# the-byte-bender/GraphAudio

Hardware: AMD Instinct MI355X
Metric: rendered frames/sec @48kHz, 1024-voice convolver graph (higher is better)
Workload: dtype f32

## Files before the change

graphaudio_amd/csrc/ga_api.cpp:

```cpp
#include <algorithm>
#include <cstring>

#include <execinfo.h>
#include <signal.h>
#include <unistd.h>

#include "ga_engine.hpp"

using namespace ga;

static void ga_segv_handler(int sig) {
  void* frames[64];
  int n = backtrace(frames, 64);
  const char msg[] = "\n[graphaudio_hip] fatal signal, native backtrace:\n";
  (void)!write(2, msg, sizeof(msg) - 1);
  backtrace_symbols_fd(frames, n, 2);
  signal(sig, SIG_DFL);
  raise(sig);
}
__attribute__((constructor)) static void ga_install_handler() {
  const char* e = getenv("GA_BACKTRACE");
  if (e && e[0] == '1') signal(SIGSEGV, ga_segv_handler);
}

struct ga_context {
  Context c;
  explicit ga_context(int sr) : c(sr) {}
};

namespace {
template <class F>
int guardRO(ga_context* h, F&& f) {
  if (!h) return GA_ERR_INVALID_ARGUMENT;
  try {
    f(h->c);
    return GA_OK;
  } catch (const Err& e) {
    h->c.lastError = e.msg;
    return e.code;
  } catch (const std::bad_alloc&) {
    h->c.lastError = "out of host memory";
    return GA_ERR_OUT_OF_MEMORY;
  } catch (const std::exception& e) {
    h->c.lastError = e.what();
    return GA_ERR_INVALID_OPERATION;
  } catch (...) {
    h->c.lastError = "unknown error";
    return GA_ERR_INVALID_OPERATION;
  }
}
template <class F>
int guard(ga_context* h, F&& f) {
  if (h) h->c.apiEpoch++;
  return guardRO(h, std::forward<F>(f));
}
float clampf(float v, float mn, float mx) {
  if (v < mn) return mn;
  if (v > mx) return mx;
  return v;
}
void addEvent(ParamS& p, const ParamEvent& e) {
  size_t lo = 0, hi = p.events.size();
  while (lo < hi) {
    size_t mid = (lo + hi) >> 1;
    if (e.time < p.events[mid].time) hi = mid; else lo = mid + 1;
  }
  p.events.insert(p.events.begin() + lo, e);
}
}

int64_t Context::chunkLimit(int64_t) {
    int64_t limit = maxChunkBlocks;
    {
      size_t freeB = 0, totalB = 0;
      if (hipMemGetInfo(&freeB, &totalB) == hipSuccess) {
        double perBlock = 0, fixedBytes = 0;
        int convRowsMax = 0;
        for (auto& g : groups) convRowsMax = std::max(convRowsMax, (int)((g->rows.size() + 127) / 128 * 128));
        perBlock += (double)convRowsMax * kBins * 4.0 * 4.0;
        int tailMax = kCoarseMaxP;
        for (auto& np : nodes)
          if (np->type == GA_NODE_CONVOLVER)
            if (const ConvolverS& cv = rec<ConvolverS>(*np); cv.ir && cv.convPath == 4) tailMax = std::max(tailMax, cv.ir->coarseP);
        for (auto& np : nodes) {
          if (np->type != GA_NODE_CONVOLVER) continue;
          const ConvolverS& cv = rec<ConvolverS>(*np);
          if (cv.ir && cv.convPath == 4) {
// ... 12 lines not shown
        budget += (double)(coarseX.bytes + coarseY.bytes + coarseM.bytes);
        int64_t byMem = (int64_t)(std::max(budget - fixedBytes, 0.0) / std::max(perBlock, 1.0));
        limit = std::max<int64_t>(1, std::min<int64_t>(limit, byMem));
      }
    }
  return limit;
}

void Context::processBlocks(float* const* outPlanar, float* outInterleaved, int channels, int64_t blockCount, bool deviceOut) {
  if (blockCount < 0) fail(GA_ERR_OUT_OF_RANGE, "blockCount");
  if (disposed) fail(GA_ERR_DISPOSED, "context disposed");
  flushHandOver();
  if (outInterleaved || outPlanar == nullptr) {
    if (channels < 1 || channels > 32) fail(GA_ERR_OUT_OF_RANGE, "channels");
    if (!outInterleaved) fail(GA_ERR_INVALID_ARGUMENT, "Buffer too small for interleaved output.");
  } else if (channels < 0 || channels > 32) {
    fail(GA_ERR_OUT_OF_RANGE, "channels");
  }
  GA_HIP(hipSetDevice(device));
  const hipMemcpyKind kind = deviceOut ? hipMemcpyDeviceToDevice : hipMemcpyDeviceToHost;
  int64_t doneBlocks = 0;
  while (doneBlocks < blockCount) {
    int64_t nblk = std::min(blockCount - doneBlocks, chunkLimit(blockCount - doneBlocks));
    runChunk(nblk, nullptr);
    const int64_t done = chunkBlocksDone;
    if (done <= 0) fail(GA_ERR_INVALID_OPERATION, "render made no progress");
    const int64_t base = doneBlocks * kBlock;
    if (outInterleaved) {
      float* stage = outInterleaved + base * channels;
      if (!deviceOut) {
        size_t need = (size_t)done * kBlock * channels * sizeof(float);
        if (ilvBytes < need) {
          if (ilvDev) {
            GA_HIP(hipStreamSynchronize(stream));
            dfree(ilvDev, ilvBytes);
          }
          ilvBytes = need + need / 4;
          ilvDev = (float*)dalloc(ilvBytes);
        }
        stage = ilvDev;
      }
      for (const SegCh& sg : chunkSegCh) {
        InterleaveSrc src{};
        const int used = std::min(channels, sg.ch);
        for (int ch = 0; ch < used; ch++) src.ch[ch] = busSlabs[ch];
        launch_interleave(stream, stage, src, channels, used, sg.b0 * kBlock, (sg.b1 - sg.b0) * kBlock);
      }
      if (!deviceOut)
        GA_HIP(hipMemcpyAsync(outInterleaved + base * channels, ilvDev, (size_t)done * kBlock * channels * sizeof(float), kind, stream));
    } else {
      for (const SegCh& sg : chunkSegCh) {
        const int used = std::min(channels, sg.ch);
        for (int ch = 0; ch < used; ch++)
          if (outPlanar[ch])
            GA_HIP(hipMemcpyAsync(outPlanar[ch] + base + sg.b0 * kBlock, busSlabs[ch] + sg.b0 * kBlock,
                                  sizeof(float) * (size_t)(sg.b1 - sg.b0) * kBlock, kind, stream));
      }
    }
    GA_HIP(hipStreamSynchronize(stream));
    doneBlocks += done;
  }
  if (blockCount > 0) freeRetired();
  stats.device_bytes_in_use = devBytes;
}

void Context::render(float* const* out, int channels, int64_t frameCount, int64_t startIndex, bool deviceOut) {
  if (channels == 0 || !out) fail(GA_ERR_INVALID_ARGUMENT, "Output buffer must have at least one channel.");
  if (frameCount <= 0) fail(GA_ERR_OUT_OF_RANGE, "Frame count must be positive.");
  if (startIndex < 0) fail(GA_ERR_OUT_OF_RANGE, "Start index must be non-negative.");
  if (channels < 0 || channels > 32) fail(GA_ERR_OUT_OF_RANGE, "channelIndex");
  for (int ch = 0; ch < channels; ch++)
    if (!out[ch]) fail(GA_ERR_INVALID_ARGUMENT, "Channel buffer is null.");
  if (disposed) fail(GA_ERR_DISPOSED, "context disposed");
  GA_HIP(hipSetDevice(device));
  const hipMemcpyKind kind = deviceOut ? hipMemcpyDeviceToDevice : hipMemcpyDeviceToHost;
  struct Pipelined {
    Context& c;
    const bool callerAsync;
    explicit Pipelined(Context& cc) : c(cc), callerAsync(cc.asyncMode) { c.asyncMode = true; }
    ~Pipelined() { c.asyncMode = callerAsync; }
  } pipelined(*this);
  struct Drain {
    Context& c;
    const bool blocking;
    ~Drain() {
      if (blocking && c.stream) (void)hipStreamSynchronize(c.stream);
      if (blocking && c.copyStream) (void)hipStreamSynchronize(c.copyStream);
    }
  } drain{*this, !pipelined.callerAsync};
  int64_t written = 0;
  if (cachedFrames > 0) {
    if (channels > cachedCh) fail(GA_ERR_OUT_OF_RANGE, "channelIndex");
    int toCopy = (int)std::min<int64_t>(cachedFrames, frameCount);
    for (int ch = 0; ch < channels; ch++)
      GA_HIP(hipMemcpyAsync(out[ch] + startIndex, cacheDev + (size_t)ch * kBlock + (kBlock - cachedFrames), sizeof(float) * toCopy,
                            kind, stream));
    if (!asyncMode) GA_HIP(hipStreamSynchronize(stream));
    written = toCopy;
    cachedFrames -= toCopy;
  }
  while (written < frameCount) {
    int64_t need = frameCount - written;
    int64_t nblk = (need + kBlock - 1) / kBlock;
    const int64_t limit = chunkLimit(nblk);
    nblk = std::min(nblk, limit);
    bool direct = (deviceOut || hostDirect) && need >= nblk * kBlock;
    float* tgt[32];
    for (int ch = 0; ch < channels && direct; ch++) {
      float* p = out[ch] + startIndex + written;
      if (!deviceOut) {
        hipPointerAttribute_t at{};
        if (hipPointerGetAttributes(&at, p) != hipSuccess || at.type != hipMemoryTypeHost || !at.devicePointer) {
          (void)hipGetLastError();
          direct = false;
          break;
        }
        p = (float*)at.devicePointer;
      }
      tgt[ch] = p;
      direct = (((uintptr_t)p) & 15) == 0;
    }
    struct Target {
      Context& c;
      ~Target() { std::memset(c.busTarget, 0, sizeof(c.busTarget)); }
    } target{*this};
    const bool defer = direct && !deviceOut && pipelined.callerAsync && hostDefer && ownStream;
    if (defer) {
      const size_t rowBytes = ((size_t)nblk * kBlock * sizeof(float) + 255) & ~(size_t)255;
      if (deferStageBytes < rowBytes * 32) {
        flushHandOver();
        if (deferStage) {
          GA_HIP(hipStreamSynchronize(stream));
          dfree(deferStage, deferStageBytes);
        }
        deferStageBytes = rowBytes * 32;
        deferStage = (float*)dalloc(deferStageBytes);
      }
      for (int ch = 0; ch < channels; ch++) busTarget[ch] = (float*)((char*)deferStage + (size_t)ch * (deferStageBytes / 32));
    } else if (direct) {
      for (int ch = 0; ch < channels; ch++) busTarget[ch] = tgt[ch];
    }
    runChunk(nblk, nullptr);
    if (defer)
      for (int ch = 0; ch < channels; ch++)
        pendingHandOver.push_back(HandOver{busTarget[ch], tgt[ch], out[ch] + startIndex + written, chunkBlocksDone * kBlock});
    std::memset(busTarget, 0, sizeof(busTarget));
    const int64_t done = chunkBlocksDone;
    if (done <= 0) fail(GA_ERR_INVALID_OPERATION, "render made no progress");
    if (channels > chunkMinDestCh) fail(GA_ERR_OUT_OF_RANGE, "channelIndex");
    const int64_t chunkFrames = done * kBlock;
    const int64_t toCopy = std::min(chunkFrames, need);
    if (direct) {
    } else if (!deviceOut && ownStream && pipelined.callerAsync && hostCopyStream) {
      handOverToHost(busSlabs.data(), out, channels, startIndex + written, toCopy);
    } else {
      for (int ch = 0; ch < channels; ch++)
        GA_HIP(hipMemcpyAsync(out[ch] + startIndex + written, busSlabs[ch], sizeof(float) * toCopy, kind, stream));
    }
    const int64_t excess = chunkFrames - toCopy;
    if (excess > 0) {
      cachedCh = chunkMinDestCh;
      for (int ch = 0; ch < cachedCh; ch++)
        GA_HIP(hipMemcpyAsync(cacheDev + (size_t)ch * kBlock, busSlabs[ch] + chunkFrames - kBlock, sizeof(float) * kBlock,
                              hipMemcpyDeviceToDevice, stream));
      cachedFrames = (int)excess;
    }
    if (!asyncMode) GA_HIP(hipStreamSynchronize(stream));
    written += toCopy;
  }
  if (!pipelined.callerAsync) {
    GA_HIP(hipStreamSynchronize(stream));
    harvestProfile(true);
    freeRetired();
  }
  stats.device_bytes_in_use = devBytes;
}

extern "C" {

const char* ga_strerror(int code) {
  switch (code) {
    case GA_OK: return "ok";
    case GA_ERR_INVALID_ARGUMENT: return "invalid argument";
    case GA_ERR_OUT_OF_RANGE: return "argument out of range";
    case GA_ERR_INVALID_OPERATION: return "invalid operation";
    case GA_ERR_DISPOSED: return "object disposed";
    case GA_ERR_CYCLE: return "audio graph cycle detected";
    case GA_ERR_UNSUPPORTED: return "unsupported on the device path";
    case GA_ERR_DEVICE: return "HIP device error";
    case GA_ERR_OUT_OF_MEMORY: return "out of memory";
    case GA_ERR_NO_DEVICE: return "no HIP device";
    default: return "unknown error code";
  }
}
const char* ga_version(void) { return "graphaudio-hip 0.1 (gfx950)"; }
int ga_device_count(void) {
  int n = 0;
  if (hipGetDeviceCount(&n) != hipSuccess) return 0;
  return n;
}

int ga_context_create(int sample_rate, int device_ordinal, ga_context** out) {
  if (!out) return GA_ERR_INVALID_ARGUMENT;
  if (sample_rate <= 0) return GA_ERR_OUT_OF_RANGE;
// ... 38 lines not shown
    else if (k == "coarse_tail") c.coarseTail = value != 0;
    else if (k == "coarse_tail_private") c.coarseTailPrivate = value != 0;
    else if (k == "sim_replay") c.simReplay = value != 0;
    else if (k == "twin_channels") c.twinChannels = value != 0;
    else if (k == "cycle_delay_split") c.cycleDelaySplit = value != 0;
    else if (k == "resample_fast") c.resampleFast = value != 0;
    else if (k == "rate_mod_walk") c.rateModWalk = value != 0;
    else if (k == "spatial_param_signals") c.spatialParamSignals = value != 0;
    else if (k == "spatial_occlusion") c.spatialOcclusion = value != 0;
    else if (k == "delay_flag_exact") {
      if (value != 0 && value != 1 && value != 2) fail(GA_ERR_OUT_OF_RANGE, "delay_flag_exact is 0, 1 or 2");
      c.delayFlagExact = (int)value;
    }
    else if (k == "conv_migrate") {
      if (value != 0 && value != 1) fail(GA_ERR_OUT_OF_RANGE, "conv_migrate is 0 or 1");
      c.convMigrate = value != 0;
    }
    else if (k == "libm_exact") {
      if (value != 0 && value != 1) fail(GA_ERR_OUT_OF_RANGE, "libm_exact is 0 or 1");
      c.libmExact = value != 0;
    }
    else if (k == "spatial_builtin_hrir") {
      if (value != 0 && value != 1) fail(GA_ERR_OUT_OF_RANGE, "spatial_builtin_hrir is 0 or 1");
      if (c.spatialBuiltinHrir != (value != 0)) c.spHeadEpoch++;
      c.spatialBuiltinHrir = value != 0;
    }
    else if (k == "spatial_head_radius") {
      if (!(value >= kSpatialHeadRadiusMin && value <= kSpatialHeadRadiusMax)) fail(GA_ERR_OUT_OF_RANGE, "spatial_head_radius is 0.04 .. 0.20 (metres)");
      c.spatialHeadRadius = value;
    }
    else if (k == "conv_reference_order") c.convRefOrder = (int)std::min(2.0, std::max(0.0, value));
    else if (k == "conv_ref_min_deviation") c.convRefMinDeviation = std::max(0.0, value);
    else if (k == "coarse_premix") c.coarsePremix = value != 0;
    else if (k == "coarse_long") c.coarseLong = value != 0;
    else if (k == "coarse_ext_history") c.coarseExtHist = value != 0;
    else if (k == "coarse_wide") c.coarseWide = value != 0;
    else if (k == "gain_pass_through") c.gainPassThrough = value != 0;
    else if (k == "gain_fold") c.gainFold = value != 0;
    else if (k == "coarse_mfma") c.coarseMfma = value != 0;
    else if (k == "biquad_time_split") c.biquadTimeSplit = (int)std::min(2.0, std::max(0.0, value));
    else if (k == "biquad_split_max_deviation") c.biquadSplitMaxDeviation = std::max(0.0, value);
    else if (k == "biquad_split_min_frames") c.biquadSplitMinFrames = std::max<int64_t>(2048, (int64_t)value);
    else if (k == "host_direct") c.hostDirect = value != 0;
    else if (k == "host_defer") c.hostDefer = value != 0;
    else if (k == "table_upload_kernel") c.tableUploadKernel = value != 0;
    else if (k == "comm_timeout_s") c.commTimeoutS = std::max(1.0, value);
    else if (k == "host_copy_stream") c.hostCopyStream = value != 0;
    else if (k == "coarse_min_blocks") c.coarseMinBlocks = std::max<int64_t>(1, (int64_t)value);
    else if (k == "debug_tconv_n2") c.debugTconvN2 = (int)value;
    else if (k == "mem_budget_fraction") c.memBudgetFraction = std::min(0.95, std::max(0.05, value));
    else if (k.rfind("listener_", 0) == 0) {
      static const char* const vec[4] = {"origin", "right", "up", "ahead"};
      int slot = -1;
      for (int v = 0; v < 4 && slot < 0; v++)
        for (int a = 0; a < 3 && slot < 0; a++)
          if (k == std::string("listener_") + vec[v] + "_" + "xyz"[a]) slot = v * 3 + a;
      if (slot < 0) fail(GA_ERR_INVALID_ARGUMENT, "unknown option " + k);
      c.listener[slot] = (float)value;
    }
    else fail(GA_ERR_INVALID_ARGUMENT, "unknown option " + k);
  });
}
int ga_get_stats(ga_context* ctx, ga_stats* out) {
  return guardRO(ctx, [&](Context& c) {
    if (!out) fail(GA_ERR_INVALID_ARGUMENT, "null pointer");
    c.harvestProfile(true);
    c.stats.device_bytes_in_use = c.devBytes;
    c.stats.n_nodes = (int)c.nodes.size();
    int rows = 0;
    for (auto& g : c.groups) rows += (int)g->rows.size();
    c.stats.n_conv_rows = rows;
    *out = c.stats;
  });
}
int ga_synchronize(ga_context* ctx) {
  return guardRO(ctx, [&](Context& c) { c.synchronize(); });
}
int ga_context_set_stream(ga_context* ctx, void* hip_stream) {
  return guard(ctx, [&](Context& c) {
    c.flushHandOver();
    GA_HIP(hipStreamSynchronize(c.stream));
    c.waitHostCopies();
    if (c.ownStream && c.stream) (void)hipStreamDestroy(c.stream);
    c.stream = (hipStream_t)hip_stream;
    c.ownStream = false;
  });
}

int ga_buffer_create(ga_context* ctx, const float* const* planar, int channels, int64_t frames, int sample_rate, int* out_id) {
  return guard(ctx, [&](Context& c) {
    if (!planar || !out_id) fail(GA_ERR_INVALID_ARGUMENT, "null pointer");
    if (channels < 1 || channels > 4096) fail(GA_ERR_OUT_OF_RANGE, "Channel count must be between 1 and 4096 (1 .. 32 for audio, more for an HRIR set)");
    if (frames < 0) fail(GA_ERR_OUT_OF_RANGE, "Length must be non-negative");
    if (sample_rate <= 0) fail(GA_ERR_OUT_OF_RANGE, "Sample rate must be positive");
    auto b = std::make_unique<PlayBuf>();
    b->channels = channels;
    b->length = frames;
    b->sampleRate = sample_rate;
    b->stride = (frames + 8 + 63) / 64 * 64;
    b->host.resize(channels);
    GA_HIP(hipSetDevice(c.device));
    size_t bytes = (size_t)b->stride * channels * sizeof(float);
    b->dev = c.dallocSkewed(bytes, &b->devBase, &b->devBytes);
    GA_HIP(hipMemsetAsync(b->dev, 0, bytes, c.stream));
    for (int i = 0; i < channels; i++) {
      if (!planar[i]) fail(GA_ERR_INVALID_ARGUMENT, "null channel pointer");
      b->host[i].assign(planar[i], planar[i] + frames);
      if (frames)
        GA_HIP(hipMemcpyAsync(b->dev + (size_t)i * b->stride, planar[i], sizeof(float) * frames, hipMemcpyHostToDevice, c.stream));
    }
    GA_HIP(hipStreamSynchronize(c.stream));
    c.buffers.push_back(std::move(b));
    c.bufVersion++;
    *out_id = (int)c.buffers.size() - 1;
  });
}
int ga_buffer_release(ga_context* ctx, int buffer_id) {
  return guard(ctx, [&](Context& c) {
    PlayBuf* b = c.buffer(buffer_id);
    if (!b || b->released) return;
    b->released = true;
    c.releasedPending.push_back(buffer_id);
  });
}

int ga_node_create(ga_context* ctx, int node_type, int* out_id) {
  return ga_node_create_ex(ctx, node_type, node_type == GA_NODE_DELAY ? 1.0 : 2.0, out_id);
}
int ga_node_create_ex(ga_context* ctx, int node_type, double arg, int* out_id) {
  return guard(ctx, [&](Context& c) {
    if (!out_id) fail(GA_ERR_INVALID_ARGUMENT, "null pointer");
    if (node_type == GA_NODE_DESTINATION) fail(GA_ERR_INVALID_ARGUMENT, "unknown node type");
    auto n = makeNode(node_type, (int)c.nodes.size(), arg, c.sampleRate);
    if (node_type == GA_NODE_BIQUAD) {
      BiquadS& bq = rec<BiquadS>(*n);
      c.updateBiquadCoefficients(bq, 1000.f, 1.0f, 0.f);
      bq.coefDirty = true;
    }
    *out_id = n->id;
    c.nodes.push_back(std::move(n));
  });
}
int ga_node_dispose(ga_context* ctx, int node) {
  return guard(ctx, [&](Context& c) {
// ... 466 lines not shown
```

graphaudio_amd/csrc/ga_chunk.cpp:

```cpp
#include "ga_chunk_internal.hpp"

namespace ga {

size_t slabsPerBlock(size_t slabBytes) {
  return slabBytes ? std::max<size_t>(8, std::min<size_t>(1024, ((size_t)1 << 30) / slabBytes)) : 0;
}

float* getSlab(Context& c) {
  if (c.slabFree.empty()) {
    size_t slabBytes = (size_t)c.slabFrames * sizeof(float);
    size_t count = slabsPerBlock(slabBytes);
    char* blk = (char*)c.dalloc(slabBytes * count);
    c.slabBlocks.push_back(blk);
    for (size_t i = 0; i < count; i++) {
      float* p = (float*)(blk + i * slabBytes);
      c.slabAll.push_back(p);
      c.slabFree.push_back(p);
    }
  }
  float* p = c.slabFree.back();
  c.slabFree.pop_back();
  return p;
}

void resetSlabs(Context& c, int64_t frames) {
  int64_t need = roundup(frames, 256);
  if (need > c.slabFrames) {
    GA_HIP(hipStreamSynchronize(c.stream));
    size_t oldBytes = (size_t)c.slabFrames * sizeof(float);
    for (void* p : c.slabBlocks) c.dfree(p, oldBytes * slabsPerBlock(oldBytes));
    c.slabBlocks.clear();
    c.slabAll.clear();
    c.slabFrames = need;
    c.slabGen++;
  }
  c.slabFree = c.slabAll;
}

const bool gaTiming = getenv("GA_TIMING") != nullptr;

double nowMs() {
  timespec ts;
  clock_gettime(CLOCK_MONOTONIC, &ts);
  return ts.tv_sec * 1e3 + ts.tv_nsec * 1e-6;
}

void Context::runChunk(int64_t n, float* const* bus) {
  if (faulted) fail(GA_ERR_INVALID_OPERATION, "context is faulted by an earlier render error (" + faultMsg + "); create a new context");
  chunkPhase = 0;
  try {
    const double t0 = gaTiming ? nowMs() : 0.0;
    runChunkImpl(n, bus);
    if (gaTiming) fprintf(stderr, "[ga]   chunk total on the host (incl. destructors): %.3f ms\n", nowMs() - t0);
  } catch (const Err& e) {
    if (chunkPhase > 0) {
      faulted = true;
      faultMsg = e.msg;
    }
    throw;
  } catch (...) {
    if (chunkPhase > 0) {
// ... 109 lines not shown
  }
  bool moved = false;
  for (auto& np : nodes) {
    if (!np || np->disposed || np->type != GA_NODE_SPATIAL_PANNER) continue;
    SpatialPannerS& nd = rec<SpatialPannerS>(*np);
    if (nd.irBuf >= 0 || nd.spGainBound == spHeadGainBound) continue;
    nd.spGainBound = spHeadGainBound;
    moved = true;
  }
  if (moved) graphVersion++;
  spHeadBoundVersion = graphVersion;
  spHeadBoundEpoch = spHeadEpoch;
}

void Context::fetchDeviceState() {
  for (size_t i = 0; i < deviceStateNodes.size();) {
    const int id = deviceStateNodes[i];
    NodeS* np = id < (int)nodes.size() ? nodes[id].get() : nullptr;
    const bool onDevice = np && !np->disposed &&
                          ((np->type == GA_NODE_STEREO_PANNER && rec<StereoPannerS>(*np).panOnDevice) ||
                           (np->type == GA_NODE_BIQUAD && rec<BiquadS>(*np).coefOnDevice) ||
                           (np->type == GA_NODE_SPATIAL_PANNER && rec<SpatialPannerS>(*np).spOnDevice));
    if (!onDevice) {
      deviceStateNodes[i] = deviceStateNodes.back();
      deviceStateNodes.pop_back();
      continue;
    }
    i++;
    if (!np->reachable) continue;
    if (np->type == GA_NODE_STEREO_PANNER) {
      StereoPannerS& nd = rec<StereoPannerS>(*np);
      if (!nd.params[0].events.empty() || !nd.params[0].modulation.empty()) continue;
      PanState tmp;
      GA_HIP(hipStreamSynchronize(stream));
      GA_HIP(hipMemcpy(&tmp, nd.panDev, sizeof(PanState), hipMemcpyDeviceToHost));
      nd.panLast = tmp.last_pan;
      nd.panGL = tmp.gain_l;
      nd.panGR = tmp.gain_r;
      nd.panOnDevice = false;
      apiEpoch++;
    } else if (np->type == GA_NODE_SPATIAL_PANNER) {
      SpatialPannerS& nd = rec<SpatialPannerS>(*np);
      if (spatialSignalDriven(nd)) continue;
      if (nd.spPrev.valid && nd.spCarry[nd.spCarryCur]) {
        SpatialCarry tmp;
        GA_HIP(hipStreamSynchronize(stream));
        GA_HIP(hipMemcpy(&tmp, nd.spCarry[nd.spCarryCur], sizeof(SpatialCarry), hipMemcpyDeviceToHost));
        for (int q = 0; q < 4; q++) {
          nd.spPrev.idx[q] = tmp.idx[q];
          nd.spPrev.w[q] = tmp.w[q];
        }
        nd.spPrev.g = tmp.g;
        nd.spPrev.beta = tmp.beta;
        if (nd.spEqOnDevice && nd.spDirect) {
          SpatialDirectState ds;
          GA_HIP(hipMemcpy(&ds, nd.spDirect, sizeof(SpatialDirectState), hipMemcpyDeviceToHost));
          nd.spEq = ds.prev;
          nd.spEqOpen = (ds.open[0] ? 1 : 0) | (ds.open[1] ? 2 : 0);
        }
      }
      nd.spEqOnDevice = false;
      nd.spOnDevice = false;
      apiEpoch++;
    } else {
      BiquadS& nd = rec<BiquadS>(*np);
      if (!nd.bqDyn) continue;
      bool automated = false;
      for (auto& p : nd.params) automated = automated || !p.events.empty() || !p.modulation.empty();
      if (!automated) {
        BiquadDynState tmp;
        GA_HIP(hipStreamSynchronize(stream));
        GA_HIP(hipMemcpy(&tmp, nd.bqDyn, 24, hipMemcpyDeviceToHost));
        nd.b0 = tmp.b0; nd.b1 = tmp.b1; nd.b2 = tmp.b2; nd.a1 = tmp.a1; nd.a2 = tmp.a2;
        nd.coefDirty = tmp.dirty != 0;
        nd.coefOnDevice = false;
        apiEpoch++;
      }
    }
  }
}

void Context::chunkSimulate(ChunkRun& r) {
  std::vector<int>& topo = r.topo;
  int64_t& n = r.n;
  std::vector<double>& bt = r.bt;
  std::vector<int>& srcIds = r.srcIds;
  std::vector<SrcPlanOut>& srcPlans = r.srcPlans;
  r.tmTopo = nowMs();
  bt.assign(n + 1, 0.0);
  bt[0] = currentTime;
  const double increment = (double)kBlock / sampleRate;
  for (int64_t i = 0; i < n; i++) bt[i + 1] = bt[i] + increment;

  std::vector<int64_t> breaks;
  for (int id : topo) {
    NodeS& nd = *nodes[id];
    const bool scheduled = nd.type == GA_NODE_CONSTANT_SOURCE || nd.type == GA_NODE_OSCILLATOR;
    if (nd.type != GA_NODE_BUFFER_SOURCE && !scheduled) continue;
    if (r.srcIndex.empty()) r.srcIndex.assign(nodes.size(), -1);
    r.srcIndex[id] = (int)srcIds.size();
    srcIds.push_back(id);
    const RateModIn* rm = (id < (int)r.rmOf.size() && r.rmOf[id] >= 0) ? &r.rmIn[r.rmOf[id]] : nullptr;
    srcPlans.push_back(scheduled ? planScheduled(*this, nd, n, bt) : planSource(*this, rec<BufferSourceS>(nd), n, bt, rm));
    for (const SrcSpan& sp : schedOf(nd).spans)
// ... 173 lines not shown
      r.segs.push_back(std::move(sg));
    }
    lastHash = prevHash;
    if (n < (int64_t)bt.size() - 1) {
      bt.resize(n + 1);
      for (int id : r.streamIds) streamReplay(rec<StreamSourceS>(*nodes[id]), n, bt, false);
    }
  }
  if (r.pre && !r.pre->preCh0.empty() && !r.pre->preSnap.empty())
    for (int id : r.pre->topo)
      for (size_t o = 0; o < nodes[id]->outputs.size(); o++) nodes[id]->outputs[o].bufCh = r.pre->preSnap.back()[(size_t)r.pre->preRow[id] + o].bufCh;
  if (r.stage != 1) chunkMinDestCh = minDestCh;
  r.tmSim = nowMs();

}

void Context::chunkResources(ChunkRun& r) {
  const int64_t frames = r.n * kBlock;
  for (int id : r.topo) {
    if (nodes[id]->type != GA_NODE_DELAY) continue;
    DelayS& nd = rec<DelayS>(*nodes[id]);
    nd.delayLoaded = false;
    int rings = std::max(nd.delayRings, 2);
    for (const Segment& sg : r.segs)
      for (const NodeSeg& ns : sg.nodes)
        if (ns.id == id) rings = std::max(rings, ns.ins[0].bufCh);
    nd.delayRings = rings;
    const size_t maxD = (size_t)nd.maxDelaySamples;
    if (nd.delayHistRings < rings) {
      float* nh = (float*)dalloc(maxD * rings * sizeof(float));
      GA_HIP(hipMemsetAsync(nh, 0, maxD * rings * sizeof(float), stream));
      if (nd.delayHist) {
        GA_HIP(hipMemcpyAsync(nh, nd.delayHist, maxD * nd.delayHistRings * sizeof(float), hipMemcpyDeviceToDevice, stream));
        GA_HIP(hipStreamSynchronize(stream));
        dfree(nd.delayHist, maxD * nd.delayHistRings * sizeof(float));
      }
      nd.delayHist = nh;
      nd.delayHistRings = rings;
    }
    const int64_t cap = roundup(frames, 4096);
    if (nd.delayCap < cap || nd.delayLineRings < rings) {
      if (nd.delayLine) {
        GA_HIP(hipStreamSynchronize(stream));
        dfree(nd.delayLine, (maxD + (size_t)nd.delayCap) * nd.delayLineRings * sizeof(float));
      }
      nd.delayCap = std::max(nd.delayCap, cap);
      nd.delayLineRings = rings;
      nd.delayLine = (float*)dalloc((maxD + (size_t)nd.delayCap) * rings * sizeof(float));
    }
    nd.delayW.assign(rings, 0);
    nd.delayR.assign(rings, 0);
  }

  if (r.stage != 2) resetSlabs(*this, frames);
  if (zerosLen < frames) {
    if (zeros) {
      GA_HIP(hipStreamSynchronize(stream));
      dfree(zeros, (size_t)zerosLen * 4);
    }
    zerosLen = roundup(frames, 4096);
    zeros = (float*)dalloc((size_t)zerosLen * 4);
    GA_HIP(hipMemsetAsync(zeros, 0, (size_t)zerosLen * 4, stream));
  }
  if (busCapFrames < frames) {
    GA_HIP(hipStreamSynchronize(stream));
    for (float* p : busSlabs) dfree(p, (size_t)busCapFrames * 4);
    busSlabs.clear();
    busCapFrames = roundup(frames, 4096);
  }
  while ((int)busSlabs.size() < 32 && (int)busSlabs.size() < std::max(destOutCh, 2)) busSlabs.push_back((float*)dalloc((size_t)busCapFrames * 4));
  {
    int mx = 0;
    for (auto& sg : r.segs)
      if (r.stage != 1) mx = std::max(mx, sg.nodes.back().outCh);
    while ((int)busSlabs.size() < mx) busSlabs.push_back((float*)dalloc((size_t)busCapFrames * 4));
  }

}

void Context::chunkExecute(ChunkRun& r) {
  int64_t& n = r.n;
  Exec& ex = *r.ex;
  r.tmPlan = nowMs();
  if (!pendingHandOver.empty()) {
    std::vector<HandOver> hv;
    hv.swap(pendingHandOver);
    hipStream_t st = stream;
    ex.plan.launches.insert(ex.plan.launches.begin(), Plan::L{[hv, st](uint8_t*) {
      for (const HandOver& h : hv) GA_HIP(hipMemcpyAsync(h.dst_host, h.src, sizeof(float) * (size_t)h.n, hipMemcpyDeviceToHost, st));
    }, LK_OTHER, 0.0, 0.0});
  }
  ex.trajOffFinal = ex.plan.putv(ex.traj);
  ex.spatialJobsOff = ex.plan.putv(ex.spatialJobs);
  size_t tbytes = ex.plan.host.size();
  const int slot = asyncMode ? (int)(chunkSeq & 1) : 0;
  void*& thost = slot ? tablesHostB : tablesHost;
  size_t& thostBytes = slot ? tablesHostBBytes : tablesHostBytes;
  if (asyncMode && chunkDone[slot]) GA_HIP(hipEventSynchronize(chunkDone[slot]));
  if (thostBytes < tbytes) {
    if (thost) {
      GA_HIP(hipStreamSynchronize(stream));
      (void)hipHostFree(thost);
    }
    thostBytes = (tbytes + tbytes / 4 + 4096 + 15) & ~(size_t)15;
    GA_HIP(hipHostMalloc(&thost, thostBytes, hipHostMallocDefault));
  }
  ensure(tables, std::max(tablesHostBytes, tablesHostBBytes));
  std::memcpy(thost, ex.plan.host.data(), tbytes);
  if (tableUploadKernel) launch_table_upload(stream, tables.p, thost, tbytes);
  else GA_HIP(hipMemcpyAsync(tables.p, thost, tbytes, hipMemcpyHostToDevice, stream));
  uint8_t* base = (uint8_t*)tables.p;

  std::vector<std::pair<hipEvent_t, hipEvent_t>> evs;
  std::vector<int> evKind;
  std::vector<double> evBytes;
  hipEvent_t evBegin = nullptr, evEnd = nullptr;
  const bool profile = profileNow;
  if (profile) {
    GA_HIP(hipEventCreate(&evBegin));
    GA_HIP(hipEventCreate(&evEnd));
    GA_HIP(hipEventRecord(evBegin, stream));
  }
  for (auto& l : ex.plan.launches) {
    hipEvent_t e0 = nullptr, e1 = nullptr;
    if (profile) {
      GA_HIP(hipEventCreate(&e0));
      GA_HIP(hipEventCreate(&e1));
      GA_HIP(hipEventRecord(e0, stream));
    }
    l.fn(base);
    if (profile) {
      GA_HIP(hipEventRecord(e1, stream));
      evs.push_back({e0, e1});
      evKind.push_back(l.kind);
      evBytes.push_back(l.bytes);
    }
    if (l.kind == GA_STAGE_COARSE_SECTION) continue;
    stats.kernel_launches++;
    if (l.kind >= 0 && l.kind < 16) {
      stats.stage_launches[l.kind]++;
      stats.stage_bytes[l.kind] += l.bytes;
      stats.stage_flops[l.kind] += l.flops;
    }
  }
  for (auto& x : extraProf) {
    evs.push_back({x.e0, x.e1});
    evKind.push_back(x.kind);
    evBytes.push_back(x.bytes);
  }
  extraProf.clear();
  if (profile) GA_HIP(hipEventRecord(evEnd, stream));
  GA_HIP(hipGetLastError());
  r.tmLaunch = nowMs();
  if (profileNow) pendingProf.push_back(ProfBatch{evBegin, evEnd, std::move(evs), std::move(evKind), std::move(evBytes)});
  if (asyncMode) {
    if (!chunkDone[slot]) GA_HIP(hipEventCreateWithFlags(&chunkDone[slot], hipEventDisableTiming));
    GA_HIP(hipEventRecord(chunkDone[slot], stream));
    harvestProfile(false);
  } else {
    GA_HIP(hipStreamSynchronize(stream));
    harvestProfile(true);
  }
  chunkSeq++;
  if (gaTiming)
    fprintf(stderr, "[ga]   host detail: topo %.2f, sources %.2f, sim %.2f | resources %.2f, params %.2f, exec %.2f ms\n", r.tmTopo - r.tm0,
            r.tmSrc - r.tmTopo, r.tmSim - r.tmSrc, r.tmRes - r.tmSim, r.tmPre - r.tmRes, r.tmPlan - r.tmPre);
  if (gaTiming)
    fprintf(stderr, "[ga] chunk %lld blocks: sim %.2f ms, plan %.2f ms, enqueue %.2f ms, wait %.2f ms\n", (long long)n, r.tmSim - r.tm0,
            r.tmPlan - r.tmSim, r.tmLaunch - r.tmPlan, nowMs() - r.tmLaunch);

}

void Context::chunkCommit(ChunkRun& r) {
  int64_t& n = r.n;
  std::vector<double>& bt = r.bt;
  std::vector<int>& srcIds = r.srcIds;
  for (size_t i = 0; i < srcIds.size(); i++) {
    SrcPlanOut& po = r.srcPlans[i];
    if (nodes[srcIds[i]]->type != GA_NODE_BUFFER_SOURCE) {
      SchedState& s = schedOf(*nodes[srcIds[i]]);
      if (po.gone && po.goneAt <= n) {
        if (!s.endedRaised) endedQueue.push_back(srcIds[i]);
        s.endedRaised = true;
        if (po.goneAt == n) pending.push_back([this, id = srcIds[i]]() { doDispose(id); });
      }
      continue;
    }
    BufferSourceS& s = rec<BufferSourceS>(*nodes[srcIds[i]]);
    if (s.spans.empty()) continue;
    int64_t firstPlay = -1;
    for (const SrcSpan& sp : s.spans)
      if ((sp.phase == SRC_PLAY || sp.phase == SRC_END) && firstPlay < 0) firstPlay = sp.b0;
    if (firstPlay < 0 || firstPlay >= n) continue;
    int64_t lastProcessed = n;
    if (po.gone && po.goneAt <= n) lastProcessed = po.goneAt;
    int64_t played = lastProcessed - firstPlay;
    PlayBuf* pb = s.bufId >= 0 ? buffers[s.bufId].get() : nullptr;
    bool rate1 = true;
    if (pb) rate1 = sourceGeom(*this, s, *pb).effectiveRate == 1.0;
    if (s.gsr && s.gsrWalked >= 0) {
      if (played == s.gsrWalked) {
        s.playbackPosition = s.gsrTail.pp;
// ... 132 lines not shown
  r1.tm0 = r.tm0;
  r1.maxDepth = r.maxDepth;
  r1.maxLevel = r.maxLevel;
  r1.rateMods = r.rateMods;
  r1.coneRoots = std::move(r.coneRoots);
  r1.probeDelays = r.probeDelays;
  r1.loopProbe = r.loopProbe;
  if (r.loopProbe) r1.stage1 = r.stage1;
  const std::vector<char>& stage1 = r.stage1;
  for (int id : r.topo)
    if (stage1[id]) r1.topo.push_back(id);
  lastSegStable = false;
  chunkSimulate(r1);
  chunkResources(r1);
  r1.tmRes = nowMs();
  bqSplitUsed = 0;
  r1.ex = std::make_unique<Exec>(*this, r1.n, r1.segs);
  r1.ex->outViews.resize(r1.segs.size());
  r1.ex->plan.host.resize(16);
  chunkStaleSeed(r1);
  curveListTopoSize = ~(size_t)0;
  chunkParamCurves(r1);
  chunkConvScratch(r1);
  r1.tmPre = nowMs();
  for (int d = 0; d <= r1.maxDepth; d++) {
    chunkPlanNodes(r1, d);
    chunkPlanConvolvers(r1, d);
  }
  chunkDelayCommit(r1);
  chunkRateProbe(r1);
  chunkExecute(r1);
  if (r1.waited) {
    const double tw0 = nowMs();
    GA_HIP(hipStreamSynchronize(stream));
    if (gaTiming) fprintf(stderr, "[ga]   two-stage chunk: stage 1 wait %.3f ms\n", nowMs() - tw0);
  }
  for (int id : r1.probeDelays) {
    DelayS& d = rec<DelayS>(*nodes[id]);
    bool read = false;
    for (DelayS::DelaySpan& sp : d.delaySpans) {
      if (sp.word < 0) continue;
      const int32_t v = r1.onsetWords[sp.word];
      if (v != std::numeric_limits<int32_t>::max()) sp.onset = v;
      read = true;
    }
    d.delayAudible = !d.delaySpans.empty() && d.delaySpans.back().onset != std::numeric_limits<int64_t>::max();
    if (read) stats.delay_flags_read++;
    if (r.loopProbe && !d.outputs.empty()) d.outputs[0].silent = !d.delayAudible;
  }

  r.stage = 2;
  r.n = r1.n;
  r.pre = &r1;
  r.rmOf = std::move(r1.rmOf);
  r.rmIn = std::move(r1.rmIn);
  {
    std::vector<int> rest;
    rest.reserve(r.topo.size() - r1.topo.size());
    for (int id : r.topo)
      if (!stage1[id]) rest.push_back(id);
    r.topo.swap(rest);
  }
  chunkSimulate(r);
  chunkResources(r);
  r.tmRes = nowMs();
  bqSplitUsed = 0;
  r.ex = std::make_unique<Exec>(*this, r.n, r.segs);
// ... 77 lines not shown
    DelayS& d = rec<DelayS>(*nodes[id]);
    for (size_t k = 0; k < d.delaySpans.size(); k++) {
      DelayS::DelaySpan& sp = d.delaySpans[k];
      const int64_t end = std::min<int64_t>(k + 1 < d.delaySpans.size() ? d.delaySpans[k + 1].b0 : n, n);
      sp.word = -1;
      if (sp.rise < 0 || sp.rise >= end || sp.ch < 1) continue;
      bool fused = false;
      for (size_t q = 0; q < ex.delayProbeNode.size(); q++)
        if (ex.delayProbeNode[q] == id) fused = true;
      if (fused) {
        sp.word = (int)nwords++;
        continue;
      }
      DelayOnsetJob oj{};
      oj.nrows = std::min(sp.ch, kDelayOnsetRows);
      for (int ch = 0; ch < oj.nrows; ch++) oj.rows[ch] = ex.nodeOut(id, ch);
      oj.first = (int32_t)sp.rise;
      oj.count = (int32_t)(end - sp.rise);
      sp.word = (int)nwords++;
      onsetWord.push_back(sp.word);
      onsets.push_back(oj);
    }
  }
  const size_t onsetOff = (size_t)roundup((int64_t)(ratesBytes + walks.size() * sizeof(GsrWalkOut)), 16);
  const size_t readBytes = nwords == 0 ? ratesBytes + walks.size() * sizeof(GsrWalkOut)
                                       : (size_t)roundup((int64_t)(onsetOff + nwords * sizeof(int32_t)), 16);
  r.waited = readBytes > 0;
  if (!r.waited) return;
  size_t descCount = 0;
  for (const GsrWalkJob& j : walks) descCount += (size_t)j.nrel + 1;
  const size_t devBytes = readBytes + descCount * sizeof(GsrBlock);
  if (rateModDevBytes < devBytes) {
    if (rateModDev) {
      GA_HIP(hipStreamSynchronize(stream));
      dfree(rateModDev, rateModDevBytes);
    }
    rateModDevBytes = devBytes + devBytes / 2 + 4096;
    rateModDev = dalloc(rateModDevBytes);
  }
  if (rateModHostBytes < readBytes) {
    if (rateModHost) (void)hipHostFree(rateModHost);
    rateModHostBytes = readBytes + readBytes / 2 + 4096;
    GA_HIP(hipHostMalloc(&rateModHost, rateModHostBytes, hipHostMallocDefault));
  }
  float* ratesDev = (float*)rateModDev;
  GsrWalkOut* outsDev = (GsrWalkOut*)((char*)rateModDev + ratesBytes);
  GsrBlock* descDev = (GsrBlock*)((char*)rateModDev + readBytes);
  const float* ratesHost = (const float*)rateModHost;
  const GsrWalkOut* outsHost = (const GsrWalkOut*)((const char*)rateModHost + ratesBytes);
  size_t d0 = 0;
  for (size_t w = 0; w < walks.size(); w++) {
    GsrWalkJob& j = walks[w];
    j.rates = ratesDev + (size_t)walkMod[w] * n;
    j.desc = descDev + d0;
    j.out = outsDev + w;
    d0 += (size_t)j.nrel + 1;
  }
  r.rmOf.assign(nodes.size(), -1);
  r.rmIn.assign(nm, RateModIn{});
  for (int k = 0; k < nm; k++) {
    RateModIn& m = r.rmIn[k];
    m.rates = ratesHost + (size_t)k * n;
    if (walkOf[k] >= 0) {
      const GsrWalkJob& j = walks[walkOf[k]];
      m.walk = outsHost + walkOf[k];
      m.desc = j.desc;
      m.nrel = j.nrel;
// ... 44 lines not shown
```

graphaudio_amd/csrc/ga_coarse.hip:

```cpp
#include "ga_kernels.hpp"
#include "ga_fft16.hpp"

#include <hip/hip_runtime.h>

#include <algorithm>
#include <atomic>
#include <string>
#include <type_traits>
#include <utility>
#include <cstdio>
#include <cstdlib>

namespace ga {

struct LdsLimit {
  std::atomic<uint64_t> done{0};
  void raise(const void* kern, size_t need, const char* what) {
    int dev = 0;
    (void)hipGetDevice(&dev);
    const uint64_t bit = 1ull << (dev & 63);
    if (done.load(std::memory_order_relaxed) & bit) return;
    if (hipFuncSetAttribute(kern, hipFuncAttributeMaxDynamicSharedMemorySize, 160 * 1024) == hipSuccess) {
      done.fetch_or(bit);
      return;
// ... 1201 lines not shown
  const CoarseHistJob J = jobs[blockIdx.y];
  const bool wide = (((uintptr_t)J.old_hist | (uintptr_t)J.in | (uintptr_t)J.new_hist) & 15) == 0;
  if (wide) {
    for (int64_t i = 4 * ((int64_t)blockIdx.x * blockDim.x + threadIdx.x); i < J.hist_len; i += 4 * (int64_t)gridDim.x * blockDim.x) {
      const int64_t sidx = i + J.n;
      v4f v = v4f{0.f, 0.f, 0.f, 0.f};
      if (sidx < J.hist_len) {
        if (J.old_hist) v = ldg4(J.old_hist + sidx);
      } else if (J.in) {
        v = ldg4(J.in + (sidx - J.hist_len));
      }
      stg4(J.new_hist + i, v);
    }
    return;
  }
  for (int64_t i = (int64_t)blockIdx.x * blockDim.x + threadIdx.x; i < J.hist_len; i += (int64_t)gridDim.x * blockDim.x) {
    const int64_t sidx = i + J.n;
    float v = 0.f;
    if (sidx < J.hist_len) v = J.old_hist ? ldg1(J.old_hist + sidx) : 0.f;
    else if (J.in) v = ldg1(J.in + (sidx - J.hist_len));
    stg1(J.new_hist + i, v);
  }
}
#ifndef GA_PREMIX_AHEAD
#define GA_PREMIX_AHEAD 8
#endif
#ifndef GA_PREMIX_WAVES
#define GA_PREMIX_WAVES 4
#endif
#ifndef GA_PREMIX_NT
#define GA_PREMIX_NT 0
#endif
constexpr int kPremixAhead = GA_PREMIX_AHEAD, kPremixWaves = GA_PREMIX_WAVES;
#ifndef GA_PREMIX_WORDS
#define GA_PREMIX_WORDS 1
#endif
#ifndef GA_PREMIX_COPY_WGS
#define GA_PREMIX_COPY_WGS 8
#endif
constexpr int kPremixCopyWgs = GA_PREMIX_COPY_WGS;
constexpr int kPremixWords = GA_PREMIX_WORDS, kPremixTile = 256 * kPremixWords;
struct Kahan4 {
  v4f s, c;
  __device__ __forceinline__ void add(v4f x) {
#ifdef GA_PREMIX_PLAIN
    s += x;
    return;
#endif
    const v4f y = x - c, t = s + y;
    c = (t - s) - y;
    s = t;
  }
};
template <bool ALIGNED, bool CARRY>
__device__ __forceinline__ void premix_stream(const PremixJob& J, const PremixTerm* __restrict terms, int t0, int t1, int lane,
                                              const uint32_t (&off)[kPremixWords], const bool (&keep)[kPremixWords],
                                              const uint32_t (&coff)[kPremixWords], Kahan4 (&acc)[kPremixWords]) {
  typedef const GA_GLOBAL char* gcp;
  typedef GA_GLOBAL char* gp;
  auto fetch = [&](gcp in, uint32_t o) -> v4f {
    if (ALIGNED) return GA_PREMIX_NT ? __builtin_nontemporal_load((const GA_GLOBAL v4f*)(in + o)) : *(const GA_GLOBAL v4f*)(in + o);
    const GA_GLOBAL float* p = (const GA_GLOBAL float*)(in + o);
    return v4f{p[0], p[1], p[2], p[3]};
  };
  auto put = [&](gp car, uint32_t o, v4f x) {
    if (GA_PREMIX_NT >= 2) __builtin_nontemporal_store(x, (GA_GLOBAL v4f*)(car + o));
    else *(GA_GLOBAL v4f*)(car + o) = x;
  };
  for (int base = t0; base < t1; base += 64) {
    const int nb = min(64, t1 - base);
    uint64_t pin = 0, pcar = 0;
    if (lane < nb) {
      const GA_GLOBAL PremixTerm* T = (const GA_GLOBAL PremixTerm*)terms + (J.term0 + base + lane);
      pin = (uint64_t)(uintptr_t)T->in;
      if (CARRY) pcar = (uint64_t)(uintptr_t)T->carry;
    }
    const int pin_lo = (int)(uint32_t)pin, pin_hi = (int)(uint32_t)(pin >> 32), pc_lo = (int)(uint32_t)pcar, pc_hi = (int)(uint32_t)(pcar >> 32);
    auto in_of = [&](int j) {
      return (gcp)(uintptr_t)(((uint64_t)(uint32_t)__builtin_amdgcn_readlane(pin_hi, j) << 32) | (uint32_t)__builtin_amdgcn_readlane(pin_lo, j));
    };
    auto carry_of = [&](int j) {
      return (gp)(uintptr_t)(((uint64_t)(uint32_t)__builtin_amdgcn_readlane(pc_hi, j) << 32) | (uint32_t)__builtin_amdgcn_readlane(pc_lo, j));
    };
    int j = 0;
    for (; j + kPremixAhead <= nb; j += kPremixAhead) {
      v4f x[kPremixAhead][kPremixWords];
#pragma unroll
      for (int u = 0; u < kPremixAhead; u++) {
        gcp in = in_of(j + u);
#pragma unroll
        for (int w = 0; w < kPremixWords; w++) x[u][w] = fetch(in, off[w]);
      }
#pragma unroll
      for (int u = 0; u < kPremixAhead; u++) {
        if (CARRY) {
          gp car = carry_of(j + u);
#pragma unroll
          for (int w = 0; w < kPremixWords; w++)
            if (car && keep[w]) put(car, coff[w], x[u][w]);
        }
#pragma unroll
        for (int w = 0; w < kPremixWords; w++) acc[w].add(x[u][w]);
      }
    }
    for (; j < nb; j++) {
      gcp in = in_of(j);
      gp car = CARRY ? carry_of(j) : nullptr;
#pragma unroll
      for (int w = 0; w < kPremixWords; w++) {
        const v4f x = fetch(in, off[w]);
        if (CARRY && car && keep[w]) put(car, coff[w], x);
        acc[w].add(x);
      }
    }
  }
}
__global__ __launch_bounds__(64 * kPremixWaves) void coarse_premix_kernel(const PremixJob* __restrict jobs, const PremixTerm* __restrict terms) {
  __shared__ v4f part[kPremixWaves - 1][2][kPremixWords][64];
  const PremixJob J = jobs[blockIdx.y];
  if (J.flags & 4) {
    if (blockIdx.x >= (unsigned)kPremixCopyWgs) return;
    const GA_GLOBAL v4f* src = (const GA_GLOBAL v4f*)terms[J.term0].in;
    GA_GLOBAL v4f* dst = (GA_GLOBAL v4f*)J.out;
    const int64_t nw = J.n / 4, step = (int64_t)kPremixCopyWgs * blockDim.x * 2;
    for (int64_t i = (int64_t)blockIdx.x * blockDim.x * 2 + threadIdx.x; i < nw; i += step) {
      const int64_t i2 = i + blockDim.x;
      const v4f a = src[i], b = i2 < nw ? src[i2] : a;
      dst[i] = a;
      if (i2 < nw) dst[i2] = b;
    }
    return;
  }
  const int64_t tile0 = (int64_t)blockIdx.x * kPremixTile;
  if (tile0 >= J.n) return;
  const int lane = threadIdx.x & 63, wv = __builtin_amdgcn_readfirstlane(threadIdx.x >> 6);
  int64_t f[kPremixWords];
  bool live[kPremixWords], keep[kPremixWords];
  uint32_t off[kPremixWords], coff[kPremixWords];
  Kahan4 acc[kPremixWords];
#pragma unroll
  for (int w = 0; w < kPremixWords; w++) {
    f[w] = tile0 + (int64_t)(w * 64 + lane) * 4;
    live[w] = f[w] < J.n;
    keep[w] = live[w] && f[w] >= J.carry_from;
    off[w] = live[w] ? (uint32_t)(f[w] * 4) : 0u;
    coff[w] = (uint32_t)((f[w] - J.carry_from) * 4);
    acc[w] = Kahan4{v4f{0.f, 0.f, 0.f, 0.f}, v4f{0.f, 0.f, 0.f, 0.f}};
  }
  const int per = ((J.nterms + kPremixWaves - 1) / kPremixWaves + kPremixAhead - 1) / kPremixAhead * kPremixAhead;
  const int t0 = min(J.nterms, wv * per), t1 = min(J.nterms, t0 + per);
  const bool carry_here = (J.flags & 2) && tile0 + kPremixTile > J.carry_from;
  if (J.flags & 1) {
    if (carry_here) premix_stream<true, true>(J, terms, t0, t1, lane, off, keep, coff, acc);
    else premix_stream<true, false>(J, terms, t0, t1, lane, off, keep, coff, acc);
  } else {
    if (carry_here) premix_stream<false, true>(J, terms, t0, t1, lane, off, keep, coff, acc);
    else premix_stream<false, false>(J, terms, t0, t1, lane, off, keep, coff, acc);
  }
  if (wv > 0) {
#pragma unroll
    for (int w = 0; w < kPremixWords; w++) {
      part[wv - 1][0][w][lane] = acc[w].s;
      part[wv - 1][1][w][lane] = acc[w].c;
    }
  }
  __syncthreads();
  if (wv == 0) {
#pragma unroll
    for (int w = 0; w < kPremixWords; w++) {
#pragma unroll
      for (int q = 0; q < kPremixWaves - 1; q++) {
        acc[w].add(part[q][0][w][lane]);
        acc[w].add(-part[q][1][w][lane]);
      }
      if (live[w]) stg4(J.out + f[w], acc[w].s);
    }
  }
}
const char* launch_coarse_premix(hipStream_t s, const PremixJob* jobs_dev, int njobs, const PremixTerm* terms_dev, int64_t max_n) {
  if (njobs <= 0 || max_n <= 0) return "";
  const int64_t gx = (max_n + kPremixTile - 1) / kPremixTile;
  if (gx > 0x7fffffff || max_n >= ((int64_t)1 << 29)) launch_fail("coarse pre-mix: chunk too long");
  for (int j0 = 0; j0 < njobs; j0 += 32768)
    hipLaunchKernelGGL(coarse_premix_kernel, dim3((unsigned)gx, std::min(32768, njobs - j0)), dim3(64 * kPremixWaves), 0, s, jobs_dev + j0, terms_dev);
  return "coarse_premix_kernel";
}

void launch_coarse_hist(hipStream_t s, const CoarseHistJob* jobs_dev, int njobs, int64_t max_len) {
  if (njobs <= 0 || max_len <= 0) return;
  const int gx = (int)std::min<int64_t>((max_len / 4 + 255) / 256, 64);
  for (int j0 = 0; j0 < njobs; j0 += 32768)
    hipLaunchKernelGGL(coarse_hist_kernel, dim3(gx, std::min(32768, njobs - j0)), dim3(256), 0, s, jobs_dev + j0);
}

__global__ __launch_bounds__(256) void table_upload_kernel(v4f* __restrict dst, const v4f* __restrict src, size_t n16) {
  for (size_t i = (size_t)blockIdx.x * 256 + threadIdx.x; i < n16; i += (size_t)gridDim.x * 256) ((GA_GLOBAL v4f*)dst)[i] = ((const GA_GLOBAL v4f*)src)[i];
}
void launch_table_upload(hipStream_t s, void* dst, const void* src_pinned, size_t bytes) {
  const size_t n16 = (bytes + 15) / 16;
  if (!n16) return;
  const unsigned grid = (unsigned)std::min<size_t>((n16 + 255) / 256, 64);
  hipLaunchKernelGGL(table_upload_kernel, dim3(grid), dim3(256), 0, s, (v4f*)dst, (const v4f*)src_pinned, n16);
}

}
```

graphaudio_amd/csrc/ga_comm.cpp:

```cpp
#include <dlfcn.h>

#include <cstring>
#include <mutex>

#include <chrono>
#include <thread>

#include "ga_engine.hpp"

#if __has_include(<rccl/rccl.h>)
#include <rccl/rccl.h>
static_assert(NCCL_UNIQUE_ID_BYTES == GA_COMM_ID_BYTES, "include/graphaudio_hip.h: GA_COMM_ID_BYTES != NCCL_UNIQUE_ID_BYTES");
static_assert(sizeof(ncclUniqueId) == GA_COMM_ID_BYTES, "ncclUniqueId is passed by value as GA_COMM_ID_BYTES bytes");
static_assert((int)ncclSuccess == 0 && (int)ncclInProgress == 7, "restated ncclResult_t values");
static_assert((int)ncclFloat32 == 7 && (int)ncclSum == 0, "restated ncclDataType_t / ncclRedOp_t values");
#endif

namespace ga {

namespace {
constexpr int kNcclSuccess = 0, kNcclInProgress = 7, kNcclFloat32 = 7, kNcclSum = 0;
struct UniqueId {
  char internal[GA_COMM_ID_BYTES];
};
// ... 63 lines not shown
    UniqueId uid;
    std::memcpy(&uid, id, sizeof(uid));
    void* c = nullptr;
    check(r, r.CommInitRank(&c, nRanks, uid, rank), "ncclCommInitRank");
    comm = c;
  }
  commRanks = nRanks;
  commRank = rank;
}

void Context::commInfo(int* nRanks, int* rank, int* usesRccl) {
  if (!nRanks || !rank || !usesRccl) fail(GA_ERR_INVALID_ARGUMENT, "null pointer");
  *nRanks = 1;
  *rank = 0;
  *usesRccl = 0;
  if (!comm) return;
  Rccl& r = rccl();
  if (!r.CommCount || !r.CommUserRank) fail(GA_ERR_UNSUPPORTED, "the RCCL library lacks ncclCommCount / ncclCommUserRank");
  check(r, r.CommCount(comm, nRanks), "ncclCommCount");
  check(r, r.CommUserRank(comm, rank), "ncclCommUserRank");
  *usesRccl = 1;
}

void Context::commAbort() {
  if (!comm) return;
  Rccl& r = rccl();
  if (r.CommAbort) (void)r.CommAbort(comm);
  else if (r.CommDestroy) (void)r.CommDestroy(comm);
  comm = nullptr;
  commDead = true;
}

void Context::commWait() {
  if (!comm) {
    GA_HIP(hipStreamSynchronize(stream));
    return;
  }
  Rccl& r = rccl();
  const auto t0 = std::chrono::steady_clock::now();
  for (;;) {
    const hipError_t q = hipStreamQuery(stream);
    if (q == hipSuccess) return;
    if (q != hipErrorNotReady) GA_HIP(q);
    (void)hipGetLastError();
    int async = kNcclSuccess;
    if (r.CommGetAsyncError && r.CommGetAsyncError(comm, &async) == kNcclSuccess && async != kNcclSuccess && async != kNcclInProgress) {
      const std::string what = r.GetErrorString ? r.GetErrorString(async) : "RCCL error";
      commAbort();
      fail(GA_ERR_DEVICE, "the communicator failed (a peer rank aborted or died): " + what);
    }
    if (std::chrono::duration<double>(std::chrono::steady_clock::now() - t0).count() > commTimeoutS) {
      commAbort();
      fail(GA_ERR_DEVICE, "timed out waiting for the sharded render's collective (option comm_timeout_s)");
    }
    std::this_thread::sleep_for(std::chrono::microseconds(200));
  }
}

void Context::commDestroy() {
  if (comm) {
    try {
      if (stream) commWait();
    } catch (...) {
    }
  }
  if (comm) {
    Rccl& r = rccl();
    if (r.CommDestroy) (void)r.CommDestroy(comm);
    comm = nullptr;
  }
  commDead = false;
  commRanks = 0;
  commRank = 0;
  if (reduceBuf) {
    dfree(reduceBuf, reduceBytes);
    reduceBuf = nullptr;
    reduceBytes = 0;
  }
}

void Context::renderReduce(float* const* out, int channels, int64_t frames, int64_t start, int root) {
  if (commRanks < 1) fail(GA_ERR_INVALID_OPERATION, "ga_comm_init has not been called on this context");
  if (commDead) fail(GA_ERR_INVALID_OPERATION, "the communicator was aborted after an error; ga_comm_destroy and ga_comm_init again");
  if (root < 0 || root >= commRanks) fail(GA_ERR_OUT_OF_RANGE, "root");
  if (channels < 1 || channels > 32) fail(GA_ERR_OUT_OF_RANGE, "channelIndex");
  if (frames <= 0) fail(GA_ERR_OUT_OF_RANGE, "Frame count must be positive.");
  if (start < 0) fail(GA_ERR_OUT_OF_RANGE, "Start index must be non-negative.");
  const bool isRoot = commRank == root;
  if (isRoot) {
    if (!out) fail(GA_ERR_INVALID_ARGUMENT, "Output buffer must have at least one channel.");
    for (int ch = 0; ch < channels; ch++)
      if (!out[ch]) fail(GA_ERR_INVALID_ARGUMENT, "Channel buffer is null.");
  }
  GA_HIP(hipSetDevice(device));
  const size_t need_ = (size_t)channels * (size_t)frames * sizeof(float);
  if (reduceBytes < need_) {
    flushHandOver();
    if (reduceBuf) {
      GA_HIP(hipStreamSynchronize(stream));
      dfree(reduceBuf, reduceBytes);
    }
    reduceBytes = need_ + need_ / 8;
    reduceBuf = (float*)dalloc(reduceBytes);
  }
  float* rows[32];
  for (int ch = 0; ch < channels; ch++) rows[ch] = reduceBuf + (size_t)ch * frames;
  const bool callerAsync = asyncMode;
  asyncMode = true;
  try {
    render(rows, channels, frames, 0, true);
    if (comm) {
      Rccl& r = rccl();
      check(r, r.Reduce(reduceBuf, reduceBuf, (size_t)channels * frames, kNcclFloat32, kNcclSum, root, comm, stream), "ncclReduce");
    }
    if (isRoot) {
      float* devAlias[32];
      bool locked = callerAsync && hostDefer && ownStream && (frames % 4) == 0;
      for (int ch = 0; ch < channels && locked; ch++) {
        hipPointerAttribute_t at{};
        if (hipPointerGetAttributes(&at, out[ch] + start) != hipSuccess || at.type != hipMemoryTypeHost || !at.devicePointer ||
            (((uintptr_t)at.devicePointer) & 15)) {
          (void)hipGetLastError();
          locked = false;
        } else {
          devAlias[ch] = (float*)at.devicePointer;
        }
      }
      if (locked) {
        for (int ch = 0; ch < channels; ch++) pendingHandOver.push_back(HandOver{rows[ch], devAlias[ch], out[ch] + start, frames});
      } else if (callerAsync && ownStream && hostCopyStream) {
        handOverToHost(rows, out, channels, start, frames);
      } else {
// ... 19 lines not shown
```

graphaudio_amd/csrc/ga_engine.cpp:

```cpp
#include "ga_engine.hpp"

#include <algorithm>
#include <cstdio>
#include <cstring>

namespace ga {

void launch_fail(const char* what) { fail(GA_ERR_INVALID_OPERATION, std::string("internal: ") + what); }

void* Context::dalloc(size_t bytes) {
  void* p = nullptr;
  if (bytes == 0) bytes = 256;
  GA_HIP(hipMalloc(&p, bytes));
  devBytes += (int64_t)bytes;
  return p;
}
float* Context::dallocSkewed(size_t bytes, void** base, size_t* total) {
  *total = bytes + 64 * 1024;
  *base = dalloc(*total);
  return (float*)((char*)*base + (size_t)(skewSeq++ % 64) * 1024);
}
double Context::biquadDeviation(const float* coefs, int nsec) {
  std::vector<float> key(coefs, coefs + 5 * nsec);
  uint64_t h = 1469598103934665603ull;
// ... 104 lines not shown
}
float* Context::bqSplitAlloc(size_t floats) {
  const size_t bytes = (floats * sizeof(float) + 63) & ~(size_t)63;
  if (bytes > kBqSplitBlock) fail(GA_ERR_INVALID_OPERATION, "internal: biquad split state larger than a block");
  if (bqSplitUsed / kBqSplitBlock != (bqSplitUsed + bytes - 1) / kBqSplitBlock) bqSplitUsed = (bqSplitUsed / kBqSplitBlock + 1) * kBqSplitBlock;
  const size_t blk = bqSplitUsed / kBqSplitBlock;
  while (bqSplitBlocks.size() <= blk) bqSplitBlocks.push_back((float*)dalloc(kBqSplitBlock));
  float* p = (float*)((char*)bqSplitBlocks[blk] + bqSplitUsed % kBqSplitBlock);
  bqSplitUsed += bytes;
  return p;
}
int Context::persistentBuffer(const float* p, int64_t n) {
  if (!p || n <= 0) return -1;
  if (bufSpansVersion != bufVersion) {
    bufSpans.clear();
    for (size_t i = 0; i < buffers.size(); i++)
      if (buffers[i] && buffers[i]->dev) bufSpans.push_back(BufSpan{buffers[i]->dev, buffers[i]->dev + (size_t)buffers[i]->stride * buffers[i]->channels, (int)i});
    std::sort(bufSpans.begin(), bufSpans.end(), [](const BufSpan& a, const BufSpan& b) { return a.lo < b.lo; });
    bufSpansVersion = bufVersion;
  }
  auto it = std::upper_bound(bufSpans.begin(), bufSpans.end(), p, [](const float* q, const BufSpan& s) { return q < s.lo; });
  if (it == bufSpans.begin()) return -1;
  --it;
  return (p >= it->lo && p + n <= it->hi) ? it->id : -1;
}
void Context::dfree(void* p, size_t bytes) {
  if (!p) return;
  (void)hipFree(p);
  devBytes -= (int64_t)(bytes == 0 ? 256 : bytes);
}
void Context::ensure(DevArena& a, size_t bytes) {
  if (a.bytes >= bytes) return;
  if (a.p) {
    GA_HIP(hipStreamSynchronize(stream));
    dfree(a.p, a.bytes);
    a.p = nullptr;
    a.bytes = 0;
  }
  size_t nb = bytes + bytes / 8;
  a.p = dalloc(nb);
  a.bytes = nb;
  GA_HIP(hipMemsetAsync(a.p, 0, nb, stream));
}

void Context::init_device(int dev) {
  int count = 0;
  if (hipGetDeviceCount(&count) != hipSuccess || count <= 0)
    fail(GA_ERR_NO_DEVICE, "no HIP device visible: libgraphaudio_hip has no CPU fallback");
  if (dev < 0 || dev >= count) fail(GA_ERR_INVALID_ARGUMENT, "device ordinal out of range");
  device = dev;
  GA_HIP(hipSetDevice(dev));
  GA_HIP(hipStreamCreateWithFlags(&stream, hipStreamNonBlocking));
  ownStream = true;
  const double pi = 3.14159265358979323846264338327950288;
  std::vector<double2> t128(64), t256(129);
  for (int j = 0; j < 64; j++) t128[j] = make_double2(std::cos(2.0 * pi * j / 128.0), -std::sin(2.0 * pi * j / 128.0));
  for (int k = 0; k <= 128; k++) t256[k] = make_double2(std::cos(2.0 * pi * k / 256.0), -std::sin(2.0 * pi * k / 256.0));
  w128 = (double2*)dalloc(sizeof(double2) * 64);
  w256 = (double2*)dalloc(sizeof(double2) * 129);
  GA_HIP(hipMemcpy(w128, t128.data(), sizeof(double2) * 64, hipMemcpyHostToDevice));
  GA_HIP(hipMemcpy(w256, t256.data(), sizeof(double2) * 129, hipMemcpyHostToDevice));
  cacheDev = (float*)dalloc(sizeof(float) * 32 * kBlock);
}

Context::~Context() {
  if (stream) (void)hipStreamSynchronize(stream);
  try {
    commDestroy();
  } catch (...) {
  }
  for (auto& b : buffers)
    if (b && b->devBase) (void)hipFree(b->devBase);
  for (auto& g : groups) {
    if (g->histR) (void)hipFree(g->histR);
    if (g->histI) (void)hipFree(g->histI);
    if (g->overlap[0]) (void)hipFree(g->overlap[0]);
    if (g->overlap[1]) (void)hipFree(g->overlap[1]);
  }
  for (auto& a : planes)
    if (a.p) (void)hipFree(a.p);
  for (auto& a : planesB)
    if (a.p) (void)hipFree(a.p);
  for (auto& a : planesBalt)
    if (a.p) (void)hipFree(a.p);
  for (auto& np : nodes) {
    if (!np) continue;
    auto drop = [](std::initializer_list<void*> ps) {
      for (void* p : ps)
        if (p) (void)hipFree(p);
    };
    switch (np->type) {
      case GA_NODE_CONVOLVER: {
        ConvolverS& cv = rec<ConvolverS>(*np);
        drop({cv.bHistR, cv.bHistI, cv.bOverlap, cv.dHistBase[0], cv.dHistBase[1], cv.dTail[0], cv.dTail[1]});
        break;
      }
      case GA_NODE_STREAM_SOURCE: {
        StreamSourceS& st = rec<StreamSourceS>(*np);
        drop({st.stWin[0], st.stWin[1]});
// ... 4 lines not shown
        drop({dl.delayHist, dl.delayLine});
        break;
      }
      case GA_NODE_OSCILLATOR: drop({rec<OscillatorS>(*np).oscPhase}); break;
      case GA_NODE_STEREO_PANNER: drop({rec<StereoPannerS>(*np).panDev}); break;
      case GA_NODE_SPATIAL_PANNER: {
        SpatialPannerS& sp = rec<SpatialPannerS>(*np);
        drop({sp.spHist[0], sp.spHist[1], sp.spCarry[0], sp.spCarry[1], sp.spDirect});
        break;
      }
      default: break;
    }
  }
  for (auto& kv : tw16) (void)hipFree(kv.second);
  if (rateModDev) (void)hipFree(rateModDev);
  if (rateModHost) (void)hipHostFree(rateModHost);
  if (coarseTw) (void)hipFree(coarseTw);
  if (tw16pw) (void)hipFree(tw16pw);
  if (copyStream) {
    (void)hipStreamSynchronize(copyStream);
    (void)hipStreamDestroy(copyStream);
    for (int k = 0; k < 2; k++) {
      if (outReady[k]) (void)hipEventDestroy(outReady[k]);
      if (outCopied[k]) (void)hipEventDestroy(outCopied[k]);
      if (outStage[k]) (void)hipFree(outStage[k]);
    }
  }
  if (stream2) {
    (void)hipStreamSynchronize(stream2);
    (void)hipStreamDestroy(stream2);
    for (auto& e : dGroupEv)
      if (e) (void)hipEventDestroy(e);
    if (dJoinEv) (void)hipEventDestroy(dJoinEv);
  }
  for (auto& x : extraProf) { (void)hipEventDestroy(x.e0); (void)hipEventDestroy(x.e1); }
  if (coarseX.p) (void)hipFree(coarseX.p);
  if (coarseY.p) (void)hipFree(coarseY.p);
  if (coarseM.p) (void)hipFree(coarseM.p);
  if (deferStage) (void)hipFree(deferStage);
  for (auto& r : retired) (void)hipFree(r.first);
  if (spHeadSet.devBase) (void)hipFree(spHeadSet.devBase);
  for (auto& kv : resamplers)
    if (kv.second->devSamples) (void)hipFree(kv.second->devSamples);
  for (auto& np : nodes)
    if (np && np->staleBuf) {
      (void)hipFree(np->staleBuf);
      (void)hipFree(np->staleNext);
    }
  for (float* p : bqSplitBlocks) (void)hipFree(p);
  if (ilvDev) (void)hipFree(ilvDev);
  if (tables.p) (void)hipFree(tables.p);
  if (tablesHost) (void)hipHostFree(tablesHost);
  if (tablesHostB) (void)hipHostFree(tablesHostB);
  for (auto& e : chunkDone)
    if (e) (void)hipEventDestroy(e);
  for (auto& b : pendingProf) {
    (void)hipEventDestroy(b.begin);
    (void)hipEventDestroy(b.end);
    for (auto& e : b.evs) { (void)hipEventDestroy(e.first); (void)hipEventDestroy(e.second); }
  }
  for (void* p : slabBlocks) (void)hipFree(p);
  for (void* p : bqBlocks) (void)hipFree(p);
  for (float* p : busSlabs) (void)hipFree(p);
  if (zeros) (void)hipFree(zeros);
  if (w128) (void)hipFree(w128);
  if (w256) (void)hipFree(w256);
  for (auto& kv : twC) (void)hipFree(kv.second);
  if (cacheDev) (void)hipFree(cacheDev);
  if (stream && ownStream) (void)hipStreamDestroy(stream);
}

void Context::executeOrPost(std::function<void()> cmd) {
  if (disposed) fail(GA_ERR_DISPOSED, "context disposed");
  if (latched && !inRender) cmd(); else pending.push_back(std::move(cmd));
}
void Context::post(std::function<void()> cmd) {
  if (disposed) fail(GA_ERR_DISPOSED, "context disposed");
  pending.push_back(std::move(cmd));
}
void Context::drain() {
  while (!pending.empty()) {
    auto cmd = std::move(pending.front());
    pending.pop_front();
    apiEpoch++;
// ... 26 lines not shown
      if (!np || np->disposed) continue;
      auto use = [&](int id) {
        if (id >= 0 && id < (int)used.size()) used[id] = 1;
      };
      switch (np->type) {
        case GA_NODE_BUFFER_SOURCE: use(rec<BufferSourceS>(*np).bufId); break;
        case GA_NODE_SPATIAL_PANNER: use(rec<SpatialPannerS>(*np).irBuf); break;
        case GA_NODE_CONVOLVER: {
          const ConvolverS& cv = rec<ConvolverS>(*np);
          use(cv.irBuf);
          for (auto& e : cv.dHistExt)
            if (e.first) use(e.second);
          break;
        }
        case GA_NODE_STREAM_SOURCE: {
          const StreamSourceS& st = rec<StreamSourceS>(*np);
          use(st.stCurrent);
          for (int id : st.stQueued) use(id);
          for (int id : st.stProcessed) use(id);
          break;
        }
        default: break;
      }
    }
    std::vector<int> keep;
    bool synced = false;
    for (int id : releasedPending) {
      if (id < 0 || id >= (int)buffers.size() || !buffers[id]) continue;
      if (used[id]) {
        keep.push_back(id);
        continue;
      }
      if (!synced && stream) {
        (void)hipStreamSynchronize(stream);
        synced = true;
      }
      PlayBuf& b = *buffers[id];
      if (b.devBase) dfree(b.devBase, b.devBytes);
      bufVersion++;
      for (auto it = irCache.begin(); it != irCache.end();)
        it = it->first.first == id ? irCache.erase(it) : std::next(it);
      buffers[id].reset();
    }
    releasedPending.swap(keep);
  }
  for (auto it = irCache.begin(); it != irCache.end();) {
    if (it->second.use_count() == 1) {
      if (stream) (void)hipStreamSynchronize(stream);
      it = irCache.erase(it);
    } else {
      ++it;
    }
  }
}

InputS* Context::inputOf(const InRef& r) {
  NodeS* n = nodes[r.node].get();
  if (r.input >= 0) return &n->inputs[r.input];
  return nullptr;
}

void Context::harvestProfile(bool wait) {
  while (!pendingProf.empty()) {
    ProfBatch& b = pendingProf.front();
    if (wait) GA_HIP(hipEventSynchronize(b.end));
    else if (hipEventQuery(b.end) != hipSuccess) { (void)hipGetLastError(); break; }
    float ms = 0;
    GA_HIP(hipEventElapsedTime(&ms, b.begin, b.end));
    stats.device_ms_total += ms;
    stats.profiled_chunks++;
    for (size_t i = 0; i < b.evs.size(); i++) {
      GA_HIP(hipEventElapsedTime(&ms, b.evs[i].first, b.evs[i].second));
      const int k = b.kinds[i];
      if (k == LK_MAC || k == LK_CMAC) stats.mac_ms_total += ms;
      else if (k == LK_FFT || k == LK_IFFT || k == LK_CFWD || k == LK_CINV || k == LK_CHIST) stats.fft_ms_total += ms;
      else if (k != GA_STAGE_COARSE_SECTION) stats.other_ms_total += ms;
      if (k >= 0 && k < 16) stats.stage_ms[k] += ms;
      (void)hipEventDestroy(b.evs[i].first);
      (void)hipEventDestroy(b.evs[i].second);
    }
    (void)hipEventDestroy(b.begin);
    (void)hipEventDestroy(b.end);
    pendingProf.pop_front();
  }
}
void Context::flushHandOver() {
  for (const HandOver& h : pendingHandOver)
    GA_HIP(hipMemcpyAsync(h.dst_host, h.src, sizeof(float) * (size_t)h.n, hipMemcpyDeviceToHost, stream));
  pendingHandOver.clear();
}
void Context::synchronize() {
  GA_HIP(hipSetDevice(device));
  flushHandOver();
  commWait();
  waitHostCopies();
  harvestProfile(true);
  freeRetired();
}
void Context::freeRetired() {
  for (auto& r : retired) dfree(r.first, r.second);
  retired.clear();
}
void Context::waitHostCopies() {
  if (!copyStream) return;
  GA_HIP(hipStreamSynchronize(copyStream));
  outPending[0] = outPending[1] = false;
}
void Context::handOverToHost(const float* const* src, float* const* out, int channels, int64_t offset, int64_t frames) {
  if (!copyStream) {
    GA_HIP(hipStreamCreateWithFlags(&copyStream, hipStreamNonBlocking));
    for (int k = 0; k < 2; k++) {
      GA_HIP(hipEventCreateWithFlags(&outReady[k], hipEventDisableTiming));
      GA_HIP(hipEventCreateWithFlags(&outCopied[k], hipEventDisableTiming));
    }
  }
  const int k = outCur;
  outCur ^= 1;
  const size_t need = (size_t)channels * (size_t)frames * sizeof(float);
  if (outStageBytes[k] < need) {
    if (outPending[k]) GA_HIP(hipEventSynchronize(outCopied[k]));
    outPending[k] = false;
    if (outStage[k]) {
      GA_HIP(hipStreamSynchronize(stream));
      dfree(outStage[k], outStageBytes[k]);
      outStage[k] = nullptr;
      outStageBytes[k] = 0;
    }
    outStage[k] = (float*)dalloc(need);
    outStageBytes[k] = need;
  }
  if (outPending[k]) GA_HIP(hipStreamWaitEvent(stream, outCopied[k], 0));
  for (int ch = 0; ch < channels; ch++)
    GA_HIP(hipMemcpyAsync(outStage[k] + (size_t)ch * frames, src[ch], sizeof(float) * (size_t)frames, hipMemcpyDeviceToDevice, stream));
  GA_HIP(hipEventRecord(outReady[k], stream));
  GA_HIP(hipStreamWaitEvent(copyStream, outReady[k], 0));
  for (int ch = 0; ch < channels; ch++)
    GA_HIP(hipMemcpyAsync(out[ch] + offset, outStage[k] + (size_t)ch * frames, sizeof(float) * (size_t)frames, hipMemcpyDeviceToHost, copyStream));
  GA_HIP(hipEventRecord(outCopied[k], copyStream));
  outPending[k] = true;
}

void Context::connectTo(int src, int out, InRef in) {
  graphVersion++;
  if (in.node == src) fail(GA_ERR_INVALID_OPERATION, "Cannot connect a node to itself");
  OutputS& o = nodes[src]->outputs[out];
  if (std::find(o.connectedInputs.begin(), o.connectedInputs.end(), in) != o.connectedInputs.end()) return;
  o.connectedInputs.push_back(in);
  if (in.input >= 0) {
    InputS& i = nodes[in.node]->inputs[in.input];
    Conn c{src, out};
    if (std::find(i.connected.begin(), i.connected.end(), c) == i.connected.end()) {
      i.connected.push_back(c);
      i.dirty = true;
    }
  } else {
    auto& m = nodes[in.node]->params[-1 - in.input].modulation;
// ... 24 lines not shown
    removeFromInput(*this, src, out, in);
  }
}
void Context::outputDisconnectAll(int src, int out) {
  graphVersion++;
  OutputS& o = nodes[src]->outputs[out];
  std::vector<InRef> ins = o.connectedInputs;
  o.connectedInputs.clear();
  for (const InRef& in : ins) removeFromInput(*this, src, out, in);
}
void Context::inputDisconnectAll(InRef in) {
  std::vector<Conn> outs;
  if (in.input >= 0) {
    outs = nodes[in.node]->inputs[in.input].connected;
  } else {
    for (auto& m : nodes[in.node]->params[-1 - in.input].modulation) outs.push_back(Conn{m.first, m.second});
  }
  for (const Conn& c : outs) disconnectFrom(c.node, c.out, in);
  if (in.input >= 0) nodes[in.node]->inputs[in.input].dirty = true;
}
void Context::doDispose(int id) {
  graphVersion++;
  NodeS& n = *nodes[id];
  if (n.disposed) return;
  n.disposed = true;
  for (int o = 0; o < (int)n.outputs.size(); o++) outputDisconnectAll(id, o);
  for (int i = 0; i < (int)n.inputs.size(); i++) {
    inputDisconnectAll(InRef{id, i});
    n.inputs[i].bufCh = 0;
  }
  for (int p = 0; p < (int)n.params.size(); p++) inputDisconnectAll(InRef{id, -1 - p});
  if (n.type == GA_NODE_DELAY) {
    DelayS& d = rec<DelayS>(n);
    if (stream) (void)hipStreamSynchronize(stream);
    if (d.delayHist) dfree(d.delayHist, (size_t)d.maxDelaySamples * d.delayHistRings * sizeof(float));
    if (d.delayLine) dfree(d.delayLine, ((size_t)d.maxDelaySamples + (size_t)d.delayCap) * d.delayLineRings * sizeof(float));
    d.delayHist = d.delayLine = nullptr;
    d.delayHistRings = d.delayLineRings = 0;
    d.delayCap = 0;
  }
  if (n.staleBuf) {
    if (stream) (void)hipStreamSynchronize(stream);
    dfree(n.staleBuf, (size_t)n.staleRows * kBlock * sizeof(float));
    dfree(n.staleNext, (size_t)n.staleRows * kBlock * sizeof(float));
    n.staleBuf = n.staleNext = nullptr;
    n.staleRows = 0;
  }
  if (n.type == GA_NODE_SPATIAL_PANNER) {
    SpatialPannerS& sp = rec<SpatialPannerS>(n);
    if (sp.spHist[0]) {
      if (stream) (void)hipStreamSynchronize(stream);
      for (float*& h : sp.spHist) {
        dfree(h, kSpatialMaxTaps * sizeof(float));
        h = nullptr;
      }
    }
    if (sp.spCarry[0]) {
      if (stream) (void)hipStreamSynchronize(stream);
      for (SpatialCarry*& h : sp.spCarry) {
        dfree(h, sizeof(SpatialCarry));
        h = nullptr;
      }
    }
    if (sp.spDirect) {
      if (stream) (void)hipStreamSynchronize(stream);
      dfree(sp.spDirect, sizeof(SpatialDirectState));
      sp.spDirect = nullptr;
    }
    sp.spOnDevice = sp.spEqOnDevice = false;
    sp.irBuf = -1;
    sp.hrirRequested = -1;
  }
  if (n.type == GA_NODE_BUFFER_SOURCE) rec<BufferSourceS>(n).bufId = -1;
  if (n.type == GA_NODE_STREAM_SOURCE) {
    StreamSourceS& st = rec<StreamSourceS>(n);
    if (st.stState != GA_STREAM_STOPPED) {
      st.stState = GA_STREAM_STOPPED;
      streamFlushToProcessed(st);
    }
  }
  if (n.type == GA_NODE_CONVOLVER) {
    ConvolverS& cv = rec<ConvolverS>(n);
    releaseConvState(cv);
    cv.ir.reset();
    cv.irBuf = -1;
  }
}

void Context::releaseConvState(ConvolverS& n) {
  graphVersion++;
  for (auto& r : n.convRows)
    if (r.group) r.group->rows[r.idx] = {-1, 0};
  n.convRows.clear();
  if (n.bHistR || n.bOverlap) {
    if (stream) (void)hipStreamSynchronize(stream);
    if (n.ir) {
      size_t hb = (size_t)n.bInCh * kBins * std::max(n.ir->P - 1, 1) * sizeof(float);
      dfree(n.bHistR, hb);
      dfree(n.bHistI, hb);
    } else {
      (void)hipFree(n.bHistR);
      (void)hipFree(n.bHistI);
    }
    dfree(n.bOverlap, (size_t)n.bSlots * 2 * kBlock * sizeof(float));
  }
  if (n.dHist[0]) {
    if (stream) (void)hipStreamSynchronize(stream);
    dfree(n.dHistBase[0], n.dHistBytes);
    dfree(n.dHistBase[1], n.dHistBytes);
    n.dHistBase[0] = n.dHistBase[1] = nullptr;
  }
  if (n.dTail[0]) {
    if (stream) (void)hipStreamSynchronize(stream);
    for (int b = 0; b < 2; b++) dfree(n.dTail[b], (size_t)n.dTailLen * n.dTailCh * sizeof(float));
  }
  n.dTail[0] = n.dTail[1] = nullptr;
  n.dTailLen = 0;
  n.dTailCh = n.dTailCur = 0;
  n.dTailSig = 0;
  n.dTailSeq = ~0ull - 1;
  n.dHist[0] = n.dHist[1] = nullptr;
  n.dHistExt.clear();
  n.dHistLen = 0;
  n.dHistCur = 0;
  n.dHistZero = true;
  n.dLeader = -1;
  n.dGroupSize = 0;
  n.everFed = false;
  fusionKeyValid = false;
  n.bHistR = n.bHistI = n.bOverlap = nullptr;
  n.bHistPlane = -1;
  n.convPath = 0;
  n.bShared = true;
  n.bHistZero = true;
  n.bOvCur = 0;
}

void Context::flushPlaneHistories(int pair) {
  std::vector<HistJobB> jobs;
  int maxh = 1;
  for (int id : bResidents[pair]) {
    ConvolverS* n = &rec<ConvolverS>(*node(id));
    if (n->bHistPlane != pair || !n->ir || !n->bHistR) continue;
    const int h = n->ir->P - 1;
    const size_t hstride = (size_t)kBins * std::max(h, 1);
    for (int c = 0; c < n->bHistNx && h > 0; c++) {
      const size_t off = (size_t)(n->bHistRow + c) * kBins * n->bHistTxb + n->bHistOff;
      jobs.push_back(HistJobB{n->bHistR + c * hstride, xPlane(pair, 0) + off, h, n->bHistTxb, h, 0});
      jobs.push_back(HistJobB{n->bHistI + c * hstride, xPlane(pair, 1) + off, h, n->bHistTxb, h, 0});
    }
    maxh = std::max(maxh, h);
    n->bHistPlane = -1;
  }
  bResidents[pair].clear();
  if (jobs.empty()) return;
  HistJobB* tab = nullptr;
  GA_HIP(hipHostMalloc((void**)&tab, jobs.size() * sizeof(HistJobB), hipHostMallocDefault));
  memcpy(tab, jobs.data(), jobs.size() * sizeof(HistJobB));
  launch_hist_copy_b(stream, tab, (int)jobs.size(), maxh);
  GA_HIP(hipGetLastError());
  GA_HIP(hipStreamSynchronize(stream));
  GA_HIP(hipHostFree(tab));
}

ConvRowRef Context::addGroupRow(const std::shared_ptr<IrSpectra>& ir, int ch, int depth, int nodeId) {
  auto key = std::make_tuple(ir.get(), ch, depth);
  ConvGroup* g;
  auto it = groupOf.find(key);
  if (it == groupOf.end()) {
    auto ng = std::make_unique<ConvGroup>();
    ng->ir = ir;
    ng->irCh = ch;
    ng->depth = depth;
    ng->P = ir->P;
    g = ng.get();
    groups.push_back(std::move(ng));
    groupOf[key] = g;
  } else {
    g = it->second;
  }
  int idx = (int)g->rows.size();
  g->rows.push_back({nodeId, ch});
  if (idx < g->rp && g->histR) {
    const int hist = g->P - 1;
    if (hist > 0) {
      GA_HIP(hipMemset2DAsync(g->histR + idx, (size_t)g->rp * 4, 0, 4, (size_t)kBins * hist, stream));
      GA_HIP(hipMemset2DAsync(g->histI + idx, (size_t)g->rp * 4, 0, 4, (size_t)kBins * hist, stream));
    }
    GA_HIP(hipMemsetAsync(g->overlap[0] + (size_t)idx * kBlock, 0, kBlock * 4, stream));
    GA_HIP(hipMemsetAsync(g->overlap[1] + (size_t)idx * kBlock, 0, kBlock * 4, stream));
  }
  return ConvRowRef{g, idx};
}

// ... 239 lines not shown
  sp->nch = nch;
  const int64_t padded = (int64_t)P * kBlock;
  std::vector<float> scaled((size_t)nch * padded, 0.f);
  for (int c = 0; c < nch; c++) {
    float scale = normalize ? normalizationScale(b->host[c].data(), b->length) : 1.0f;
    float* dst = &scaled[(size_t)c * padded];
    const float* src = b->host[c].data();
    for (int64_t i = 0; i < b->length; i++) dst[i] = src[i] * scale;
  }
  GA_HIP(hipSetDevice(device));
  const int rp = 128;
  float* dIn = (float*)dalloc(scaled.size() * sizeof(float));
  size_t planeBytes = (size_t)kBins * P * rp * sizeof(float);
  float* xr = (float*)dalloc(planeBytes);
  float* xi = (float*)dalloc(planeBytes);
  size_t hBytes = (size_t)nch * kBins * P * sizeof(float);
  sp->hBytes = hBytes;
  sp->devBytesRef = &devBytes;
  sp->hr = (float*)dalloc(hBytes);
  sp->hi = (float*)dalloc(hBytes);
  ConvRowIO* rowsDev = (ConvRowIO*)dalloc(sizeof(ConvRowIO) * nch);
  std::vector<ConvRowIO> rows(nch);
  for (int c = 0; c < nch; c++) rows[c] = ConvRowIO{dIn + (size_t)c * padded, nullptr};
  GA_HIP(hipMemcpyAsync(dIn, scaled.data(), scaled.size() * sizeof(float), hipMemcpyHostToDevice, stream));
  GA_HIP(hipMemcpyAsync(rowsDev, rows.data(), sizeof(ConvRowIO) * nch, hipMemcpyHostToDevice, stream));
  GA_HIP(hipMemsetAsync(xr, 0, planeBytes, stream));
  GA_HIP(hipMemsetAsync(xi, 0, planeBytes, stream));
  ConvPlanes pl{xr, xi, nullptr, nullptr, P, 0, rp};
  for (int t0 = 0; t0 < P; t0 += 32768) {
    int nb = std::min(32768, P - t0);
    std::vector<ConvRowIO> r2(nch);
    for (int c = 0; c < nch; c++) r2[c] = ConvRowIO{dIn + (size_t)c * padded + (size_t)t0 * kBlock, nullptr};
    if (t0 > 0) {
      GA_HIP(hipStreamSynchronize(stream));
      GA_HIP(hipMemcpy(rowsDev, r2.data(), sizeof(ConvRowIO) * nch, hipMemcpyHostToDevice));
    }
    launch_rfft_fwd(stream, rowsDev, nch, nb, t0, pl, Twiddles{w128, w256});
  }
  launch_extract_ir(stream, sp->hr, sp->hi, xr, xi, P, rp, P, nch);
  GA_HIP(hipStreamSynchronize(stream));
  GA_HIP(hipGetLastError());
  sp->taps = dIn;
  sp->tapsStride = padded;
  sp->tapsBytes = scaled.size() * sizeof(float);
  dfree(xr, planeBytes);
  dfree(xi, planeBytes);
  dfree(rowsDev, sizeof(ConvRowIO) * nch);
  irCache[key] = sp;
  return sp;
}

const float2* Context::twiddles16(int N2) {
  auto it = tw16.find(N2);
  if (it != tw16.end()) return it->second;
  const double pi = 3.14159265358979323846264338327950288;
  const int R3 = N2 / 256;
  std::vector<float2> t;
  for (int m = 1; m < 16; m++)
    for (int kk = 0; kk < 16; kk++) t.push_back(make_float2((float)std::cos(2.0 * pi * kk * m / 256), (float)-std::sin(2.0 * pi * kk * m / 256)));
  for (int m = 1; m < R3; m++)
    for (int j = 0; j < 256; j++) t.push_back(make_float2((float)std::cos(2.0 * pi * j * m / N2), (float)-std::sin(2.0 * pi * j * m / N2)));
  float2* d = (float2*)dalloc(sizeof(float2) * t.size());
  GA_HIP(hipMemcpy(d, t.data(), sizeof(float2) * t.size(), hipMemcpyHostToDevice));
  tw16[N2] = d;
  return d;
}

void Context::streamFlushToProcessed(StreamSourceS& s) {
  if (s.stCurrent >= 0) s.stProcessed.push_back(s.stCurrent);
  s.stCurrent = -1;
  while (!s.stQueued.empty()) {
    s.stProcessed.push_back(s.stQueued.front());
    s.stQueued.pop_front();
  }
  if (s.stChannels >= 0) {
    s.stRsPos = 0.0;
    s.stRsReady = 0;
    s.stWinValid = false;
  }
  s.stPos = 0;
  s.stLastRate = 0;
}

void Context::ensureOverlapStream() {
  if (stream2) return;
  GA_HIP(hipStreamCreateWithFlags(&stream2, hipStreamNonBlocking));
  for (auto& e : dGroupEv) GA_HIP(hipEventCreateWithFlags(&e, hipEventDisableTiming));
  GA_HIP(hipEventCreateWithFlags(&dJoinEv, hipEventDisableTiming));
}
const float2* Context::coarseTwab() {
  if (coarseTw) return coarseTw;
  const double pi = 3.14159265358979323846264338327950288;
  std::vector<float2> t(2 * 2049);
  for (int k = 0; k <= 2048; k++) {
    t[k] = make_float2((float)std::cos(2.0 * pi * k / 8192), (float)-std::sin(2.0 * pi * k / 8192));
    t[2049 + k] = make_float2((float)std::cos(2.0 * pi * k / 16384), (float)-std::sin(2.0 * pi * k / 16384));
  }
  coarseTw = (float2*)dalloc(sizeof(float2) * t.size());
  GA_HIP(hipMemcpy(coarseTw, t.data(), sizeof(float2) * t.size(), hipMemcpyHostToDevice));
  return coarseTw;
}
void Context::ensureCoarseSpectra(IrSpectra& ir) {
  if (ir.coarse) return;
  if (!ir.taps) fail(GA_ERR_INVALID_OPERATION, "internal: impulse response without device taps");
  const int P = (int)((ir.tapsStride + kCoarseBlock - 1) / kCoarseBlock);
  ir.coarseP = P;
  const int PS = P > kCoarseMaxP ? (P + kCoarseMaxP - 1) / kCoarseMaxP * kCoarseMaxP : P;
  ir.coarseStride = PS;
  ir.coarseBytes = (size_t)ir.nch * PS * kCoarseBins * sizeof(float2);
  ir.coarse = (float2*)dalloc(ir.coarseBytes);
  if (PS != P) GA_HIP(hipMemsetAsync(ir.coarse, 0, ir.coarseBytes, stream));
  std::vector<CoarseXRow> rows(ir.nch);
  for (int c = 0; c < ir.nch; c++) {
    CoarseXRow& r = rows[c];
    r.hist = nullptr;
    r.in = ir.taps + (size_t)c * ir.tapsStride;
    r.nvalid = ir.tapsStride;
    r.frame0 = c * PS;
    r.n_frames = P;
    r.u0 = 1;
    r.hist_len = 0;
    r.flags = 1;
    r.scale = 1.0f / 65536.0f;
    r.carry = nullptr;
    r.carry_from = 0;
  }
  CoarseXRow* rd = (CoarseXRow*)dalloc(sizeof(CoarseXRow) * rows.size());
  GA_HIP(hipMemcpy(rd, rows.data(), sizeof(CoarseXRow) * rows.size(), hipMemcpyHostToDevice));
  launch_coarse_fwd(stream, rd, ir.nch, P, P, ir.coarse, twiddles16pw(), coarseTwab());
  GA_HIP(hipGetLastError());
  GA_HIP(hipStreamSynchronize(stream));
  dfree(rd, sizeof(CoarseXRow) * rows.size());
}

const float2* Context::twiddles16pw() {
  if (tw16pw) return tw16pw;
  const double pi = 3.14159265358979323846264338327950288;
  std::vector<float2> t;
  for (int m = 1; m < 16; m++)
    for (int kk = 0; kk < 16; kk++) t.push_back(make_float2((float)std::cos(2.0 * pi * kk * m / 256), (float)-std::sin(2.0 * pi * kk * m / 256)));
  for (int m : {1, 2, 4, 8})
    for (int j = 0; j < 256; j++) t.push_back(make_float2((float)std::cos(2.0 * pi * j * m / 4096), (float)-std::sin(2.0 * pi * j * m / 4096)));
  tw16pw = (float2*)dalloc(sizeof(float2) * t.size());
  GA_HIP(hipMemcpy(tw16pw, t.data(), sizeof(float2) * t.size(), hipMemcpyHostToDevice));
  return tw16pw;
}

const float2* Context::twiddlesC(int N2) {
  auto it = twC.find(N2);
  if (it != twC.end()) return it->second;
  const double pi = 3.14159265358979323846264338327950288;
  std::vector<float2> t(N2);
  for (int j = 0; j < N2; j++) t[j] = make_float2((float)std::cos(2.0 * pi * j / N2), (float)-std::sin(2.0 * pi * j / N2));
  float2* d = (float2*)dalloc(sizeof(float2) * N2);
  GA_HIP(hipMemcpy(d, t.data(), sizeof(float2) * N2, hipMemcpyHostToDevice));
  twC[N2] = d;
  return d;
}
const float2* Context::ensureTapSpectra(IrSpectra& ir, int N2) {
  if (N2 != 1024 && N2 != 2048 && N2 != 4096) fail(GA_ERR_INVALID_OPERATION, "internal: no block-axis FFT of " + std::to_string(N2) + " points");
  float2*& h = ir.hspecN[IrSpectra::n2Index(N2)];
  if (h) return h;
  size_t bytes = (size_t)ir.nch * kBins * N2 * sizeof(float2);
  ir.hspecBytes += bytes;
// ... 82 lines not shown
```

graphaudio_amd/csrc/ga_engine.hpp:

```cpp
#pragma once
#include <cstring>
#include <initializer_list>
#include <new>
#include <hip/hip_runtime.h>

#include <algorithm>
#include <cmath>
#include <cstdint>
#include <deque>
#include <functional>
#include <limits>
#include <map>
#include <tuple>
#include <memory>
#include <string>
#include <unordered_map>
#include <vector>

#include "../../include/graphaudio_hip.h"
#include "ga_kernels.hpp"
#include "ga_gsr.hpp"
#include "ga_topology.hpp"

namespace ga {
// ... 779 lines not shown
  bool spatialSignalDriven(const NodeS& nd) const {
    if (!spatialParamSignals || nd.type != GA_NODE_SPATIAL_PANNER) return false;
    for (int p = 0; p < GA_SPATIAL_PARAM_COUNT && p < (int)nd.params.size(); p++)
      if (!nd.params[p].modulation.empty()) return true;
    return false;
  }
  bool spatialOcclusion = false;
  bool spatialBuiltinHrir = false;
  double spatialHeadRadius = kSpatialHeadRadiusDefault;
  PlayBuf spHeadSet;
  double spHeadSetRadius = 0.0;
  float spHeadGainBound = 1.f;
  uint64_t spHeadEpoch = 1;
  double spHeadBoundRadius = 0.0;
  uint64_t spHeadBoundVersion = ~0ull, spHeadBoundEpoch = 0;
  void spatialHeadBounds();
  void ensureSpatialHeadSet();
  SpatialBands spBands{};
  bool spBandsMade = false;
  int delayFlagExact = 0;
  bool rateModWalk = true;
  bool resampleFast = true;
  void assignConvPaths(const std::vector<int>& topo, int64_t chunkBlocks);
  hipStream_t copyStream = nullptr;
  bool hostCopyStream = false;
  hipEvent_t outReady[2] = {nullptr, nullptr}, outCopied[2] = {nullptr, nullptr};
  float* outStage[2] = {nullptr, nullptr};
  size_t outStageBytes[2] = {0, 0};
  bool outPending[2] = {false, false};
  int outCur = 0;
  void handOverToHost(const float* const* src, float* const* out, int channels, int64_t offset, int64_t frames);
  void waitHostCopies();
  hipStream_t stream2 = nullptr;
  hipEvent_t dGroupEv[8] = {nullptr, nullptr, nullptr, nullptr, nullptr, nullptr, nullptr, nullptr};
  hipEvent_t dJoinEv = nullptr;
  bool coarseOverlap = false;
  bool coarseTail = true;
  int convRefOrder = 1;
  double convRefMinDeviation = 2.5e-6;
  std::vector<char> refSensScratch;
  bool convMigrate = false;
  bool libmExact = false;
  struct ConvMigration {
    int id;
    const float* src[32];
  };
  std::vector<ConvMigration> convMigrations;
  void migrateConvolvers(const std::vector<int>& topo);
  void planConvMigration(ChunkRun& r);
  bool coarseTailPrivate = false;
  bool coarseCarry = true;
  bool coarseLong = true;
  bool coarsePremix = true;
  void ensureOverlapStream();
  void noteKernel(int kind, const char* name) {
    if (kind < 0 || kind >= 16 || !name || !*name) return;
    std::strncpy(stats.stage_kernel[kind], name, sizeof(stats.stage_kernel[kind]) - 1);
  }
  struct ExtraProf { hipEvent_t e0, e1; int kind; double bytes; };
  std::vector<ExtraProf> extraProf;
  std::vector<std::vector<NodeSeg>> segNodePool;
  std::vector<std::vector<Views>> viewsPool;
  DevArena coarseM;
  DevArena coarseX, coarseY;
  float2* coarseTw = nullptr;
  const float2* coarseTwab();
  float2* tw16pw = nullptr;
  const float2* twiddles16pw();
  void ensureCoarseSpectra(IrSpectra& ir);
  void planCoarseFusion(const std::vector<int>& topo, const std::vector<Segment>& segs);
  uint64_t fusionKey = 0;
  bool fusionKeyValid = false;
  void aliasBusToLeader(ChunkRun& r);
  ConvRowRef addGroupRow(const std::shared_ptr<IrSpectra>& ir, int ch, int depth, int nodeId);
  void ensureGroupState(ConvGroup& g);
  const float2* twiddlesC(int N2);
  const float2* twiddles16(int N2);
  std::map<int, float2*> tw16;
  bool useRadix16 = true;
  bool useCoarse = true;
  int64_t coarseMinBlocks = 256;
  int debugTconvN2 = 0;
  const float2* ensureTapSpectra(IrSpectra& ir, int N2);
  struct TconvLaunch { int N2, tbase, nseg; };
  std::vector<TconvLaunch> tconvPlan(int nblocks, int P) const;
  bool fft64 = false;
// ... 113 lines not shown
```

graphaudio_amd/csrc/ga_kernels.hpp:

```cpp
#pragma once
#include <hip/hip_runtime.h>
#include <stdint.h>
#include <stdlib.h>

#include "ga_spatial_geom.hpp"
#include "ga_spatial_direct.hpp"
#include "ga_spatial_head.hpp"
#include "ga_conv_rebuild.hpp"

namespace ga {

[[noreturn]] void launch_fail(const char* what);

#ifdef GA_EXPERIMENTS
inline const char* expenv(const char* name) { return getenv(name); }
#else
inline const char* expenv(const char*) { return nullptr; }
#endif

constexpr int kBlock = 128;
constexpr int kBins = 129;

struct ConvPlanes {
  float* xr;
// ... 113 lines not shown
  int yrow0;
  int shared_h;
  int u_lo, u_hi;
  int pad_;
};
struct CoarseOut {
  float* out;
  int64_t nvalid;
  int y0, ny;
  const float* tail_in;
  float* tail_out;
  int64_t tail_len;
  int n_y;
  int pad_;
};
struct CoarseHistJob {
  const float* old_hist;
  const float* in;
  float* new_hist;
  int64_t hist_len, n;
};
struct PremixTerm {
  const float* in;
  float* carry;
};
struct PremixJob {
  float* out;
  int term0, nterms;
  int64_t n;
  int64_t carry_from;
  int flags;
  int pad_;
};
const char* launch_coarse_premix(hipStream_t s, const PremixJob* jobs_dev, int njobs, const PremixTerm* terms_dev, int64_t max_n);
const char* launch_coarse_fwd(hipStream_t s, const CoarseXRow* rows_dev, int nrows, int max_frames, int run, float2* X, const float2* tw16,
                       const float2* twab, const CoarseHandOver* handover_dev = nullptr, int n_handover = 0);
const char* launch_coarse_mac(hipStream_t s, const CoarseJob* jobs_dev, int njobs, const CoarseTerm* terms_dev, const float2* X, float2* Y,
                       int y_frames, int cw, int max_t, int maxP, bool any_private, int pb, bool matrix_cores = false);
const char* launch_coarse_inv(hipStream_t s, const CoarseOut* outs_dev, int nouts, int n_t, const int* ylist_dev, const float2* Y, int y_frames,
                       const float2* tw16, const float2* twab);
void launch_coarse_hist(hipStream_t s, const CoarseHistJob* jobs_dev, int njobs, int64_t max_len);
void launch_table_upload(hipStream_t s, void* dst, const void* src_pinned, size_t bytes);

struct MixJob {
  float* out;
  int term0;
  int nterms;
  int64_t f0;
  int64_t n;
  float* out2 = nullptr;
};
void launch_mix(hipStream_t s, const MixJob* jobs_dev, int njobs, const float* const* terms_dev, int64_t max_n, bool vec4, const float* gains_dev = nullptr,
                const float* const* curves_dev = nullptr);

void launch_mix_wide(hipStream_t s, const MixJob* jobs_dev, int njobs, const float* const* terms_dev, int64_t max_n, const float* gains_dev = nullptr,
                     const float* const* curves_dev = nullptr);
constexpr int kMixWideMinTerms = 256;

struct DownmixJob {
  float* out;
  int term0;
  int nch;
  float scale;
  int64_t f0;
  int64_t n;
};
void launch_downmix(hipStream_t s, const DownmixJob* jobs_dev, int njobs, const float* const* terms_dev, int64_t max_n, const float* gains_dev = nullptr);
// ... 415 lines not shown
```

graphaudio_amd/csrc/ga_plan_conv.cpp:

```cpp
#include "ga_chunk_internal.hpp"

namespace ga {

void Context::ensureGroupState(ConvGroup& g) {
  Context& c = *this;
  int need = (int)roundup(std::max<size_t>(g.rows.size(), 1), 128);
  if (need <= g.rp) return;
  const int hist = g.P - 1;
  size_t hBytes = (size_t)kBins * std::max(hist, 1) * need * sizeof(float);
  size_t oBytes = (size_t)need * kBlock * sizeof(float);
  float* nr = (float*)c.dalloc(hBytes);
  float* ni = (float*)c.dalloc(hBytes);
  float* o0 = (float*)c.dalloc(oBytes);
  float* o1 = (float*)c.dalloc(oBytes);
  GA_HIP(hipMemsetAsync(nr, 0, hBytes, c.stream));
  GA_HIP(hipMemsetAsync(ni, 0, hBytes, c.stream));
  GA_HIP(hipMemsetAsync(o0, 0, oBytes, c.stream));
  GA_HIP(hipMemsetAsync(o1, 0, oBytes, c.stream));
  if (g.rp > 0) {
    if (hist > 0 && !g.histZero) {
      GA_HIP(hipMemcpy2DAsync(nr, (size_t)need * 4, g.histR, (size_t)g.rp * 4, (size_t)g.rp * 4, (size_t)kBins * hist,
                              hipMemcpyDeviceToDevice, c.stream));
      GA_HIP(hipMemcpy2DAsync(ni, (size_t)need * 4, g.histI, (size_t)g.rp * 4, (size_t)g.rp * 4, (size_t)kBins * hist,
                              hipMemcpyDeviceToDevice, c.stream));
    }
    GA_HIP(hipMemcpyAsync(o0, g.overlap[g.ovCur], (size_t)g.rp * kBlock * 4, hipMemcpyDeviceToDevice, c.stream));
    GA_HIP(hipStreamSynchronize(c.stream));
    size_t oldH = (size_t)kBins * std::max(hist, 1) * g.rp * sizeof(float);
    c.dfree(g.histR, oldH);
    c.dfree(g.histI, oldH);
    c.dfree(g.overlap[0], (size_t)g.rp * kBlock * 4);
    c.dfree(g.overlap[1], (size_t)g.rp * kBlock * 4);
  }
  g.histR = nr;
  g.histI = ni;
  g.overlap[0] = o0;
  g.overlap[1] = o1;
  g.ovCur = 0;
  g.rp = need;
}

void Context::planCoarseFusion(const std::vector<int>& topo, const std::vector<Segment>& segs) {
  {
    uint64_t key = hmix(graphVersion, (uint64_t)segs.size());
    for (const Segment& sg : segs) key = hmix(key, sg.hash);
    for (int id : topo) {
      if (nodes[id]->type != GA_NODE_CONVOLVER) continue;
      const ConvolverS& nd = rec<ConvolverS>(*nodes[id]);
      key = hmix(hmix(key, ((uint64_t)id << 8) | (uint64_t)nd.convPath), (uint64_t)(uintptr_t)nd.ir.get());
    }
    if (fusionKeyValid && key == fusionKey) return;
    fusionKey = key;
    fusionKeyValid = true;
  }
  std::vector<int> cand;
  for (int id : topo) {
    if (nodes[id]->type != GA_NODE_CONVOLVER) continue;
    ConvolverS& nd = rec<ConvolverS>(*nodes[id]);
    nd.dLeader = -1;
    if (!nd.ir || nd.convPath != 4) continue;
// ... 78 lines not shown
struct CoarseStage {
  Context& c;
  Exec& ex;
  const std::vector<int>& dNodes;
  const int64_t n, frames;
  const int nT;
  static constexpr int kVoicesPerJob = kCoarseJobTerms;
  struct Piece {
    int frame0, P, xrow, u0;
    IrSpectra* ir;
    int leader;
    int ncol;
    int irCh[16], outCh[16];
  };
  struct GroupInfo {
    uint64_t sig = 1469598103934665603ull;
    int maxP = 0, nIn = 0, nOut = 0;
    const void* ir0 = nullptr;
    bool oneIr = true, tail = false, carried = false, fresh = true, noHist = false;
    bool uniform = true, premix = false;
    int members = 0, nxr = 0, bInCh0 = 0, bSlots0 = 0;
    bool ts0 = false;
    int64_t hl0 = 0;
    struct Terms { std::vector<PremixTerm> in[32], hist[32]; };
    std::unique_ptr<Terms> terms;
  };
  std::vector<Views> chInOf;
  bool wideStrided = true;
  std::vector<CoarseHandOver> fwdHandOver;
  std::vector<PremixJob> pmJobs;
  std::vector<PremixTerm> pmTerms;
  size_t pmUsed = 0;
  int64_t pmMaxN = 0;
  double pmBytes = 0;
  std::vector<CoarseXRow> xrows;
  std::vector<CoarseHistJob> hjobs;
  std::vector<Piece> pieces;
  std::map<int, GroupInfo> groups;
  const bool tails;
  int frameNext = 0;
  int64_t maxHist = 0;
  double histBytes = 0;
  std::map<int, double> carryBytes;
  int nxAll = 0, G = 1;
  int gBegin[9] = {};
  std::vector<CoarseTerm> terms;
  static constexpr int kCwOf[4] = {1, 2, 4, 16};
  std::vector<CoarseJob> jobs[16][8];
  int maxT[16] = {}, maxP[16] = {};
  int pbOf[16] = {4, 4, 4, 4, 4, 4, 4, 4, 4, 4, 4, 4, 4, 4, 4, 4};
  double macBytes[16][8] = {}, macFlops[16][8] = {};
  double pmFlops = 0, invFlops = 0;
  std::map<std::pair<int, int>, std::vector<int>> outRows;
  int yNext = 0;
  std::vector<CoarseOut> outs;
  std::vector<int> ylist;
  double invBytes = 0;
  int yFrames = 0, invBlocks = 0;

  CoarseStage(Context& c_, Exec& ex_, const std::vector<int>& d, int64_t n_)
      : c(c_), ex(ex_), dNodes(d), n(n_), frames(n_ * kBlock), nT((int)((n_ * kBlock + kCoarseBlock - 1) / kCoarseBlock)), tails(c_.coarseTail) {}
  void resolveInputs();
  void classifyGroups();
  void buildRows();
  void addPieces(ConvolverS& nd, int leader, int nxr, const int* xFrame, const int* xIndex);
  void buildJobs();
// ... 158 lines not shown
      r.hist_len = (int)hl;
      r.flags = 0;
      r.scale = 1.0f;
      xFrame[ch] = frameNext;
      xIndex[ch] = (int)xrows.size();
      frameNext += r.n_frames;
      float* nextHist = nd.dHist[nd.dHistCur ^ 1] + (size_t)ch * hl;
      r.carry = nullptr;
      r.carry_from = 0;
      if (coarseHistoryStays(c, nd, ch, r.in, frames)) {
      } else if (c.coarseCarry && r.in && frames >= hl && (((uintptr_t)r.in | (uintptr_t)nextHist) & 15) == 0) {
        r.carry = nextHist;
        r.carry_from = frames - hl;
        carryBytes[(int)xrows.size()] = (double)hl * 4.0;
      } else {
        hjobs.push_back(CoarseHistJob{oldHist, r.in, nextHist, hl, frames});
        maxHist = std::max(maxHist, hl);
        histBytes += 2.0 * (double)hl * 4.0;
      }
      xrows.push_back(r);
    }
    nd.dHistCur ^= 1;
    nd.dHistZero = false;
    addPieces(nd, nd.dLeader >= 0 ? nd.dLeader : id, nxr, xFrame, xIndex);
  }
  for (auto& kv : groups) {
    GroupInfo& g = kv.second;
    if (!g.premix) continue;
    ConvolverS& ld = rec<ConvolverS>(*c.nodes[kv.first]);
    const int64_t hl = g.hl0;
    int xFrame[32], xIndex[32];
    for (int ch = 0; ch < g.nxr; ch++) {
      const size_t bytes = (size_t)(hl + frames) * sizeof(float);
      if (pmUsed + bytes > c.coarseM.bytes) fail(GA_ERR_INVALID_OPERATION, "internal: the pre-mix arena is too small for the plan");
      float* mixed = (float*)((char*)c.coarseM.p + pmUsed);
      pmUsed += (bytes + 255) & ~(size_t)255;
      auto job = [&](float* out, const std::vector<PremixTerm>& tv, int64_t len, int64_t carryFrom) {
        PremixJob j{out, (int)pmTerms.size(), 0, len, carryFrom, 1, 0};
        for (const PremixTerm& t : tv) {
          if (!t.in) continue;
          pmTerms.push_back(t);
          j.nterms++;
          if ((uintptr_t)t.in & 15) j.flags &= ~1;
          if (t.carry) j.flags |= 2;
          pmBytes += (double)len * 4.0;
          pmFlops += (double)len * 4.0;
        }
        pmJobs.push_back(j);
        pmMaxN = std::max(pmMaxN, len);
        pmBytes += (double)len * 4.0;
      };
      if (!g.terms) g.terms = std::make_unique<GroupInfo::Terms>();
      if (!g.noHist) job(mixed, g.terms->hist[ch], hl, hl);
      job(mixed + hl, g.terms->in[ch], frames, std::max<int64_t>(0, frames - hl));
      CoarseXRow r{};
      r.hist = g.noHist ? nullptr : mixed;
      r.in = mixed + hl;
      r.nvalid = frames;
      r.frame0 = frameNext;
      r.u0 = g.noHist ? 0 : -(g.maxP - 1);
      r.n_frames = (g.tail ? nT + 1 : nT) - r.u0;
      r.hist_len = (int)hl;
      r.flags = 0;
      r.scale = 1.0f;
      r.carry = nullptr;
      r.carry_from = 0;
      xFrame[ch] = frameNext;
      xIndex[ch] = (int)xrows.size();
      frameNext += r.n_frames;
      xrows.push_back(r);
    }
    addPieces(ld, kv.first, g.nxr, xFrame, xIndex);
    c.stats.coarse_premixed_signals += (int64_t)g.members * g.nxr;
  }
  if (!pmJobs.empty() && !c.pendingHandOver.empty()) {
    std::vector<PremixJob> head;
    for (const Context::HandOver& h : c.pendingHandOver) {
      head.push_back(PremixJob{h.dst_dev, (int)pmTerms.size(), 1, h.n, h.n, 1 | 4, 0});
      pmTerms.push_back(PremixTerm{h.src, nullptr});
      pmMaxN = std::max(pmMaxN, h.n);
      pmBytes += 2.0 * (double)h.n * 4.0;
    }
    pmJobs.insert(pmJobs.begin(), head.begin(), head.end());
    c.pendingHandOver.clear();
    c.stats.deferred_handovers++;
  } else if (!c.pendingHandOver.empty() && !xrows.empty()) {
    for (const Context::HandOver& h : c.pendingHandOver) fwdHandOver.push_back(CoarseHandOver{h.src, h.dst_dev, h.n});
    c.pendingHandOver.clear();
    c.stats.deferred_handovers++;
  }
  ex.flushLevel();
}

void CoarseStage::buildJobs() {
  struct Key {
    int leader, P, ncol;
    std::array<int, 16> out;
    bool operator<(const Key& o) const { return std::tie(leader, P, ncol, out) < std::tie(o.leader, o.P, o.ncol, o.out); }
  };
  std::map<Key, std::vector<const Piece*>> byKey;
  for (const Piece& pc : pieces) {
    Key k{pc.leader, pc.P, pc.ncol, {}};
    k.out.fill(-1);
    for (int j = 0; j < pc.ncol; j++) k.out[j] = pc.outCh[j];
    byKey[k].push_back(&pc);
  }
  nxAll = (int)xrows.size();
  G = !c.coarseOverlap ? 1 : (nxAll >= 256 ? 4 : (nxAll >= 64 ? 2 : 1));
  auto groupOf = [&](int xrow) { return std::min(G - 1, (int)((int64_t)xrow * G / std::max(nxAll, 1))); };
  for (int g = 0; g <= G; g++) gBegin[g] = 0;
  for (int x = 0; x < nxAll; x++) gBegin[groupOf(x) + 1] = x + 1;
  for (int g = 1; g <= G; g++) gBegin[g] = std::max(gBegin[g], gBegin[g - 1]);
  for (auto& kv : byKey) {
    const Key& k = kv.first;
    const int cw = k.ncol, ci = cw == 1 ? 0 : (cw == 2 ? 1 : (cw == 4 ? 2 : 3));
    const auto& pv = kv.second;
// ... 73 lines not shown
          continue;
        }
        jobs[cj][grp].push_back(jb_);
        maxT[cj] = std::max(maxT[cj], jb_.n_t);
        maxP[cj] = std::max(maxP[cj], k.P);
        while (k.P % pbOf[cj]) pbOf[cj] >>= 1;
        const int fread = std::max(0, std::min(jb_.u_hi, t0 + jb_.n_t - 1) - std::max(jb_.u_lo, t0 - (k.P - 1)) + 1);
        macBytes[cj][grp] += (double)jb_.n_terms * fread * kCoarseBins * 8.0 +
                             (t0 == 0 ? (double)(shared ? 1 : jb_.n_terms) * k.P * cw * kCoarseBins * 8.0 : 0.0) + (double)cw * jb_.n_t * kCoarseBins * 8.0;
        macFlops[cj][grp] += shared ? ((double)jb_.n_terms * fread * 2.0 + (double)k.P * jb_.n_t * cw * 8.0) * kCoarseBins
                                    : (double)jb_.n_terms * k.P * jb_.n_t * cw * 8.0 * kCoarseBins;
      }
    }
  }
}

void CoarseStage::buildOutputs() {
  int maxPAll = 0;
  for (auto& kv : groups)
    if (kv.second.tail) maxPAll = std::max(maxPAll, kv.second.maxP);
  yFrames = nT + maxPAll;
  invBlocks = nT;
  if (tails) {
    std::map<int, int> chOf;
    for (auto& kv : outRows) chOf[kv.first.first] = std::max(chOf[kv.first.first], kv.first.second + 1);
    for (auto& kv : groups) {
      if (!kv.second.tail) continue;
      ConvolverS& ld = rec<ConvolverS>(*c.nodes[kv.first]);
      const int64_t len = (int64_t)(kv.second.maxP + 1) * kCoarseBlock;
      const int nch = chOf.count(kv.first) ? chOf[kv.first] : 0;
      if (nch == 0) continue;
      if (!ld.dTail[0] || ld.dTailLen != len || ld.dTailCh != nch) {
        if (kv.second.carried) fail(GA_ERR_INVALID_OPERATION, "internal: a carried tail changed its shape");
        GA_HIP(hipStreamSynchronize(c.stream));
        for (int b = 0; b < 2; b++) {
          if (ld.dTail[b]) c.dfree(ld.dTail[b], (size_t)ld.dTailLen * ld.dTailCh * sizeof(float));
          ld.dTail[b] = (float*)c.dalloc((size_t)len * nch * sizeof(float));
        }
        ld.dTailLen = len;
        ld.dTailCh = nch;
        ld.dTailCur = 0;
      }
    }
  }
  for (auto& kv : outRows) {
    CoarseOut o{};
    o.out = ex.nodeOut(kv.first.first, kv.first.second);
    o.nvalid = frames;
    o.y0 = (int)ylist.size();
    o.ny = (int)kv.second.size();
    o.n_y = nT;
    if (groups[kv.first.first].tail) {
      ConvolverS& ld = rec<ConvolverS>(*c.nodes[kv.first.first]);
      const GroupInfo& gi = groups[kv.first.first];
      o.n_y = nT + gi.maxP;
      o.tail_len = ld.dTailLen;
      o.tail_in = gi.carried ? ld.dTail[ld.dTailCur] + (size_t)kv.first.second * ld.dTailLen : nullptr;
      o.tail_out = ld.dTail[ld.dTailCur ^ 1] + (size_t)kv.first.second * ld.dTailLen;
      invBlocks = std::max(invBlocks, (int)((frames + o.tail_len + kCoarseBlock - 1) / kCoarseBlock));
      invBytes += (double)o.tail_len * 4.0 * (gi.carried ? 2.0 : 1.0);
      if (gi.carried) c.stats.coarse_carried_outputs++;
    }
    ylist.insert(ylist.end(), kv.second.begin(), kv.second.end());
    outs.push_back(o);
    invBytes += (double)o.ny * o.n_y * kCoarseBins * 8.0 + (double)frames * 4.0;
    invFlops += (double)o.n_y * (kCoarseTransformFlops + (double)o.ny * 2.0 * kCoarseBins);
  }
  if (tails)
    for (auto& kv : groups) {
      ConvolverS& ld = rec<ConvolverS>(*c.nodes[kv.first]);
      if (!kv.second.tail || !ld.dTail[0]) continue;
      ld.dTailCur ^= 1;
      ld.dTailSig = kv.second.sig;
      ld.dTailSeq = c.chunkSeq;
    }
  if ((size_t)frameNext * kCoarseBins * sizeof(float2) > c.coarseX.bytes || (size_t)yNext * yFrames * kCoarseBins * sizeof(float2) > c.coarseY.bytes)
    fail(GA_ERR_INVALID_OPERATION, "internal: coarse spectra arenas are too small for the plan");

}

void CoarseStage::enqueue() {
  const int G = this->G, yFrames = this->yFrames, invBlocks = this->invBlocks, nxAll = this->nxAll;
  const double invBytes = this->invBytes, histBytes = this->histBytes;
  const size_t xo = ex.plan.putv(xrows), ho = ex.plan.putv(hjobs), to = ex.plan.putv(terms), oo = ex.plan.putv(outs), yo = ex.plan.putv(ylist);
  const size_t pjo = ex.plan.putv(pmJobs), pto = ex.plan.putv(pmTerms), fho = ex.plan.putv(fwdHandOver);
  const int nfh = (int)fwdHandOver.size();
  const int npm = (int)pmJobs.size();
  const int64_t pmMaxN = this->pmMaxN;
  const double pmBytes = this->pmBytes, pmFlops = this->pmFlops, invFlops = this->invFlops;
  struct MacLaunch { size_t off; int nj, cw, mt, mp, pb, grp; bool ap; double bytes, flops; };
  const bool matrixCores = c.coarseMfma && wideStrided;
  std::vector<MacLaunch> macs;
  for (int g = 0; g < G; g++)
    for (int i = 0; i < 16; i++) {
      if (jobs[i][g].empty()) continue;
      macs.push_back(MacLaunch{ex.plan.putv(jobs[i][g]), (int)jobs[i][g].size(), kCwOf[(i & 7) >> 1], maxT[i], maxP[i], pbOf[i], g, (i & 1) == 0,
                               macBytes[i][g], macFlops[i][g]});
      c.stats.mac_launches += 1;
    }
  hipStream_t st = c.stream;
  float2* X = (float2*)c.coarseX.p;
  float2* Y = (float2*)c.coarseY.p;
  const float2* tw16 = c.twiddles16(4096);
  const float2* twFwd = c.twiddles16pw();
  const float2* twab = c.coarseTwab();
  const int nh = (int)hjobs.size(), no = (int)outs.size();
  struct FwdLaunch { int x0, nx, maxFrames, run; double bytes, flops; };
  std::vector<FwdLaunch> fwds;
  for (int g = 0; g < G; g++) {
    FwdLaunch f{this->gBegin[g], this->gBegin[g + 1] - this->gBegin[g], 0, 1, 0.0, 0.0};
    for (int x = f.x0; x < f.x0 + f.nx; x++) {
      f.maxFrames = std::max(f.maxFrames, xrows[x].n_frames);
      f.bytes += (double)(xrows[x].n_frames + 1) * kCoarseBlock * 4.0 + (double)xrows[x].n_frames * kCoarseBins * 8.0;
      f.flops += (double)xrows[x].n_frames * kCoarseTransformFlops;
      if (auto it = carryBytes.find(x); it != carryBytes.end()) f.bytes += it->second;
    }
    while (f.run < 16 && (int64_t)nxAll * ((f.maxFrames + 2 * f.run - 1) / (2 * f.run)) >= 1024) f.run *= 2;
    if (f.run >= 8) {
      const int k = (f.maxFrames + 11) / 12;
      f.run = (f.maxFrames + k - 1) / k;
    }
    if (const char* e = expenv("GA_COARSE_RUN")) f.run = std::max(1, atoi(e));
    fwds.push_back(f);
  }
  if (G > 1) c.ensureOverlapStream();
  Context* cp = &c;
  ex.plan.add(GA_STAGE_COARSE_SECTION, [=](uint8_t* base) {
    auto timed = [&](hipStream_t sx, int kind, double bytes, double flops, const std::function<const char*()>& launch) {
      hipEvent_t e0 = nullptr, e1 = nullptr;
      if (cp->profileNow) {
        GA_HIP(hipEventCreate(&e0));
        GA_HIP(hipEventCreate(&e1));
        GA_HIP(hipEventRecord(e0, sx));
      }
      cp->noteKernel(kind, launch());
      if (cp->profileNow) {
        GA_HIP(hipEventRecord(e1, sx));
        cp->extraProf.push_back(Context::ExtraProf{e0, e1, kind, bytes});
      }
      cp->stats.kernel_launches++;
      cp->stats.stage_launches[kind]++;
      cp->stats.stage_bytes[kind] += bytes;
      cp->stats.stage_flops[kind] += flops;
    };
    hipStream_t s2 = G > 1 ? cp->stream2 : st;
    if (npm > 0)
      timed(st, LK_CPREMIX, pmBytes, pmFlops, [&] { return launch_coarse_premix(st, (const PremixJob*)(base + pjo), npm, (const PremixTerm*)(base + pto), pmMaxN); });
    for (int g = 0; g < G; g++) {
      const FwdLaunch& f = fwds[g];
      if (f.nx > 0)
        timed(st, LK_CFWD, f.bytes, f.flops, [&] {
          return launch_coarse_fwd(st, (const CoarseXRow*)(base + xo) + f.x0, f.nx, f.maxFrames, f.run, X, twFwd, twab,
                                   (const CoarseHandOver*)(base + fho), g == 0 ? nfh : 0);
        });
      if (G > 1) {
        GA_HIP(hipEventRecord(cp->dGroupEv[g], st));
        GA_HIP(hipStreamWaitEvent(s2, cp->dGroupEv[g], 0));
      }
      for (const MacLaunch& m : macs)
        if (m.grp == g)
          timed(s2, LK_CMAC, m.bytes, m.flops, [&] {
            return launch_coarse_mac(s2, (const CoarseJob*)(base + m.off), m.nj, (const CoarseTerm*)(base + to), X, Y, yFrames, m.cw, m.mt, m.mp, m.ap, m.pb,
                                     matrixCores);
          });
    }
    if (G > 1) {
      GA_HIP(hipEventRecord(cp->dJoinEv, s2));
      GA_HIP(hipStreamWaitEvent(st, cp->dJoinEv, 0));
    }
  });
  ex.plan.add(LK_CINV, [=](uint8_t* base) {
    cp->noteKernel(LK_CINV, launch_coarse_inv(st, (const CoarseOut*)(base + oo), no, invBlocks, (const int*)(base + yo), Y, yFrames, tw16, twab));
  }, invBytes, invFlops);
  const int64_t mh = maxHist;
  if (nh > 0) ex.plan.add(LK_CHIST, [=](uint8_t* base) { launch_coarse_hist(st, (const CoarseHistJob*)(base + ho), nh, mh); }, histBytes);
}
}

static void planCoarseStage(Context& c, Exec& ex, const std::vector<int>& dNodes, int64_t n) {
  CoarseStage s(c, ex, dNodes, n);
  s.resolveInputs();
  s.classifyGroups();
  s.buildRows();
  s.buildJobs();
  s.buildOutputs();
  s.enqueue();
}

void Context::aliasBusToLeader(ChunkRun& r) {
  Exec& ex = *r.ex;
  int leader = -1, nch = 0;
  for (const Segment& sg : r.segs) {
    if (sg.nodes.empty() || sg.nodes.back().id != 0 || sg.nodes.back().ins.empty()) return;
    const InSeg& is = sg.nodes.back().ins[0];
    for (const TermS& t : is.terms) {
      if (nodes[t.node]->type != GA_NODE_CONVOLVER) return;
      const ConvolverS& nd = rec<ConvolverS>(*nodes[t.node]);
      if (!nd.ir || nd.convPath != 4 || nd.dLeader < 0 || t.out != 0 || t.ch != is.bufCh) return;
      if (leader < 0) {
        leader = nd.dLeader;
        nch = is.bufCh;
      } else if (leader != nd.dLeader || nch != is.bufCh) {
        return;
      }
    }
// ... 228 lines not shown
        if (nodes[id]->type != GA_NODE_CONVOLVER) continue;
        ConvolverS& nd = rec<ConvolverS>(*nodes[id]);
        if (!nd.ir || nd.convPath != 4) continue;
        auto& pd = perDepth[nd.depth];
        pd.first += (size_t)nd.bInCh * (size_t)(nT + nd.ir->coarseP);
        pd.second += (size_t)nd.bSlots;
        int& tp = tailDepth[nd.depth];
        tp = std::max(tp, std::max(kCoarseMaxP, nd.ir->coarseP));
      }
      size_t xf = 0, yf = 0;
      for (auto& kv : perDepth) {
        xf = std::max(xf, kv.second.first);
        yf = std::max(yf, kv.second.second * (size_t)(nT + tailDepth[kv.first]));
      }
      if (xf) {
        ensure(coarseX, xf * kCoarseBins * sizeof(float2));
        ensure(coarseY, yf * kCoarseBins * sizeof(float2));
      }
      if (coarsePremix) {
        std::map<int, int> members;
        for (int id : topo) {
          if (nodes[id]->type != GA_NODE_CONVOLVER) continue;
          const ConvolverS& nd = rec<ConvolverS>(*nodes[id]);
          if (nd.ir && nd.convPath == 4) members[nd.dLeader >= 0 ? nd.dLeader : id]++;
        }
        std::map<int, size_t> pmDepth;
        for (auto& kv : members) {
          if (kv.second < 2) continue;
          const ConvolverS& ld = rec<ConvolverS>(*nodes[kv.first]);
          pmDepth[ld.depth] += (size_t)ld.bInCh * ((((size_t)(ld.dHistLen + n * kBlock) * sizeof(float)) + 255) & ~(size_t)255);
        }
        size_t pm = 0;
        for (auto& kv : pmDepth) pm = std::max(pm, kv.second);
        if (pm) ensure(coarseM, pm);
      }
    }
    bRowX = bRowY = 0;
    if (bx) {
      const size_t txb = (size_t)roundup(bHistMax, 4) + roundup(n, 16) + 16, tyb = (size_t)roundup(n, 256);
      bPairWrite = bPairCur ^ 1;
      flushPlaneHistories(bPairWrite);
      const size_t xb = bx * kBins * txb * sizeof(float);
      if (planesB[0].bytes < xb || planesBalt[0].bytes < xb) flushPlaneHistories(bPairCur);
      ensure(planesB[0], xb);
      ensure(planesB[1], xb);
      ensure(planesBalt[0], xb);
      ensure(planesBalt[1], xb);
      ensure(planesB[2], by * kBins * tyb * sizeof(float));
      ensure(planesB[3], by * kBins * tyb * sizeof(float));
    }
  }

  if (topology.hasOscillators)
  for (int id : topo) {
    if (nodes[id]->type != GA_NODE_OSCILLATOR) continue;
    OscillatorS& nd = rec<OscillatorS>(*nodes[id]);
    if (nd.oscPhase) continue;
    nd.oscPhase = (double*)dalloc(64);
    GA_HIP(hipMemsetAsync(nd.oscPhase, 0, 64, stream));
  }
}

void Context::planConvolversShared(ChunkRun& r, int , ConvPlanCtx& k) {
  int64_t& n = r.n;
  std::vector<Segment>& segs = r.segs;
  Exec& ex = *r.ex;
  auto& active = k.active; auto& tsTemps = k.tsTemps; auto& prevIns = k.prevIns; int& prevP = k.prevP; int& prevRp = k.prevRp; int& prevRows = k.prevRows;
// ... 393 lines not shown
```

graphaudio_amd/csrc/ga_plan_nodes.cpp:

```cpp
#include "ga_chunk_internal.hpp"

namespace ga {

void Context::chunkParamCurves(ChunkRun& r) {
  std::vector<int>& topo = r.topo;
  Exec& ex = *r.ex;
  if (curveListEpoch != apiEpoch || curveListGraphVersion != graphVersion || curveListTopoSize != topo.size()) {
    for (auto& e : curveList)
      if (e.first < (int)nodes.size() && nodes[e.first] && e.second < (int)nodes[e.first]->params.size()) nodes[e.first]->params[e.second].curve = nullptr;
    curveList.clear();
    for (int id : topo) {
      NodeS& nd = *nodes[id];
      for (auto& p : nd.params) p.curve = nullptr;
      if (nd.type != GA_NODE_GAIN && nd.type != GA_NODE_BIQUAD && nd.type != GA_NODE_CONSTANT_SOURCE && nd.type != GA_NODE_OSCILLATOR &&
          nd.type != GA_NODE_DELAY && nd.type != GA_NODE_STEREO_PANNER)
        continue;
      for (int pi = 0; pi < (int)nd.params.size(); pi++)
        if (!nd.params[pi].events.empty()) curveList.push_back({id, pi});
    }
    curveListEpoch = apiEpoch;
    curveListGraphVersion = graphVersion;
    curveListTopoSize = topo.size();
  }
  std::vector<ParamJob> pjobs;
// ... 678 lines not shown
  if (ns.bqDynamic) {
    auto iv = ex.resolveInput((int)si, ns, 0, false, nullptr);
    ensureBiquadState(nd);
    nd.bqTwinN = 1;
    BiquadDynJob dj{};
    for (int ch = 0; ch < ns.outCh && ch < 32; ch++) {
      dj.in[ch] = iv[ch];
      dj.out[ch] = ex.nodeOut(ns.id, ch);
      ov[ch] = dj.out[ch];
    }
    dj.fcurve = ex.paramView((int)si, ns, 0);
    dj.qcurve = ex.paramView((int)si, ns, 1);
    dj.gcurve = ex.paramView((int)si, ns, 2);
    dj.fval = nd.params[0].value;
    dj.qval = nd.params[1].value;
    dj.gval = nd.params[2].value;
    dj.channels = ns.outCh;
    dj.filter_type = nd.filterType;
    if (nd.coefOnDevice && nd.coefDirty) {
      dj.filter_type |= 0x100;
      nd.coefDirty = false;
    }
    dj.nyquist = sampleRate / 2.f;
    dj.sample_rate = (float)sampleRate;
    dj.state = nd.bqDyn;
    dj.b0 = sg.b0;
    dj.nblocks = nb;
    if (!nd.coefOnDevice) {
      BiquadDynState init{};
      init.b0 = nd.b0; init.b1 = nd.b1; init.b2 = nd.b2; init.a1 = nd.a1; init.a2 = nd.a2;
      init.dirty = nd.coefDirty ? 1 : 0;
      nd.coefDirty = false;
      GA_HIP(hipMemcpyAsync(nd.bqDyn, &init, 24, hipMemcpyHostToDevice, stream));
      GA_HIP(hipStreamSynchronize(stream));
      nd.coefOnDevice = true;
      deviceStateNodes.push_back(ns.id);
    }
    ex.bqDynJobs.push_back(dj);
    return;
  }
  if (absorbedBy.get(ns.id) >= 0) return;
  SmallVec<const NodeSeg*, kMaxBiquadSections> chain{&ns};
  while (true) {
    const NodeSeg* h = chain.front();
    if (h->ins[0].terms.size() != 1) break;
    int up = h->ins[0].terms[0].node;
    if (absorbedBy.get(up) != h->id) break;
    chain.insert_front(segNode.find(up));
  }
  auto iv = ex.resolveInput((int)si, *chain.front(), 0, false, nullptr);
  for (const NodeSeg* cn : chain) {
    BiquadS& cnd = rec<BiquadS>(*nodes[cn->id]);
    ensureBiquadState(cnd);
  }
  int G = 1;
  float coefs[5 * kMaxBiquadSections];
  if (biquadTimeSplit && nf >= biquadSplitMinFrames) {
    const int64_t lanes = 64 * 1024, heads = std::max(levelBqHeads, 1);
    G = (int)std::max<int64_t>(1, std::min<int64_t>({(lanes + heads - 1) / heads, nf / 1024, 256}));
    int q = 0;
    for (const NodeSeg* cn : chain) {
      coefs[5 * q] = cn->b0; coefs[5 * q + 1] = cn->b1; coefs[5 * q + 2] = cn->b2; coefs[5 * q + 3] = cn->a1; coefs[5 * q + 4] = cn->a2;
      q++;
    }
    if (biquadTimeSplit == 1 && biquadDeviation(coefs, (int)chain.size()) > biquadSplitMaxDeviation) G = 1;
  }
  int64_t K = G > 1 ? ((nf + G - 1) / G + 31) / 32 * 32 : nf;
// ... 235 lines not shown
        fprintf(stderr, "[stale] chunk %llu node %d type %d row %d: views %d (of %zu nodes) view %p alive %d scale %g curve %p\n", (unsigned long long)chunkSeq, id,
                nd.type, rw, haveViews ? (int)lastViews[id].size() : -1, lastViews.size(), (const void*)src, (int)alive(src), g, (const void*)sj.curve);
#endif
    }
  };
  for (int id : topology.staleProducers) {
    NodeS& nd = *nodes[id];
    if (nd.staleBuf && nd.staleSeq + 1 == chunkSeq) continue;
    if (nd.prevReachable || !nd.staleBuf) keepLastBlock(nd);
  }
  for (int id : topology.staleLeavers) {
    NodeS& nd = *nodes[id];
    if (nd.staleBuf && nd.staleSeq + 1 == chunkSeq) continue;
    if (!haveLast || id >= (int)lastViews.size()) continue;
    bool any = false;
    for (const float* v : lastViews[id]) any = any || v != nullptr;
    if (any || nd.staleBuf) keepLastBlock(nd);
  }
  topology.staleLeavers.clear();
  hipStream_t st = stream;
  ex.flush(jobs, LK_OTHER, nullptr, [=](const StaleJob* t, int nj, int64_t, uint8_t*) { launch_stale_copy(st, t, nj); });
}

void Context::chunkStaleCommit(ChunkRun& r) {
  if (topology.staleProducers.empty()) return;
  Exec& ex = *r.ex;
  std::vector<StaleJob> jobs;
  const int si = (int)r.segs.size() - 1;
  for (int id : topology.staleProducers) {
    NodeS& nd = *nodes[id];
    const int rows = nd.type == GA_NODE_CHANNEL_SPLITTER ? std::max<int>(1, (int)nd.outputs.size()) : 32;
    if (!nd.staleBuf || nd.staleRows < rows) {
      if (nd.staleBuf) {
        GA_HIP(hipStreamSynchronize(stream));
        dfree(nd.staleBuf, (size_t)nd.staleRows * kBlock * sizeof(float));
        dfree(nd.staleNext, (size_t)nd.staleRows * kBlock * sizeof(float));
      }
      nd.staleRows = rows;
      nd.staleBuf = (float*)dalloc((size_t)rows * kBlock * sizeof(float));
      nd.staleNext = (float*)dalloc((size_t)rows * kBlock * sizeof(float));
      GA_HIP(hipMemsetAsync(nd.staleBuf, 0, (size_t)rows * kBlock * sizeof(float), stream));
      GA_HIP(hipMemsetAsync(nd.staleNext, 0, (size_t)rows * kBlock * sizeof(float), stream));
    }
    const Views* ov = (si >= 0 && id < (int)ex.outViews[si].size()) ? &ex.outViews[si][id] : nullptr;
    const float g = si >= 0 ? ex.scaleOf(si, id) : 1.f;
    for (int rw = 0; rw < nd.staleRows; rw++) {
      const float* src = (ov && rw < (int)ov->size() && (*ov)[rw]) ? (*ov)[rw] + (r.n - 1) * kBlock : nullptr;
      jobs.push_back(StaleJob{nd.staleNext + (size_t)rw * kBlock, src, g, 0});
    }
    std::swap(nd.staleBuf, nd.staleNext);
    nd.staleSeq = chunkSeq;
  }
  hipStream_t st = stream;
  ex.flush(jobs, LK_OTHER, nullptr, [=](const StaleJob* t, int nj, int64_t, uint8_t*) { launch_stale_copy(st, t, nj); });
}

void Context::chunkDelayCommit(ChunkRun& r) {
  Exec& ex = *r.ex;
  for (int id : r.topo) {
    if (nodes[id]->type != GA_NODE_DELAY) continue;
    DelayS& nd = rec<DelayS>(*nodes[id]);
    if (!nd.delayLoaded) continue;
    const size_t maxD = (size_t)nd.maxDelaySamples, pitch = maxD + (size_t)nd.delayCap;
    for (int r = 0; r < nd.delayHistRings; r++) {
      if (nd.delayW[r] == 0) continue;
      float* dst = nd.delayHist + (size_t)r * maxD;
      const float* src = nd.delayLine + (size_t)r * pitch + nd.delayW[r];
// ... 8 lines not shown
```

Baseline: 1.222 billion.

## Run coarse convolution tail on second stream overlapping next chunk's premix

Adds an optional tail-stream mode. When a chunk's plan is only a coarse section plus inverse FFT, the forward, MAC and inverse stages go to a second stream, so the next chunk's host work and premix can overlap them. To make that safe it double-buffers the premix arena and the device table arena by chunk parity, and replaces stream syncs with a syncStream helper that also joins the tail. The premix kernel is also rewritten to split each job across a configurable number of workgroups per CU, with handover copies folded into the same grid. The extra events, cross-stream dependencies and arena double-buffering add complexity and ordering risk.

```diff
diff --git a/graphaudio_amd/csrc/ga_api.cpp b/graphaudio_amd/csrc/ga_api.cpp
--- a/graphaudio_amd/csrc/ga_api.cpp
+++ b/graphaudio_amd/csrc/ga_api.cpp
@@ -52,7 +52,10 @@
 template <class F>
 int guard(ga_context* h, F&& f) {
   if (h) h->c.apiEpoch++;
-  return guardRO(h, std::forward<F>(f));
+  return guardRO(h, [&](Context& c) {
+    c.joinTail();
+    f(c);
+  });
 }
 float clampf(float v, float mn, float mx) {
   if (v < mn) return mn;
@@ -131,7 +134,7 @@
         size_t need = (size_t)done * kBlock * channels * sizeof(float);
         if (ilvBytes < need) {
           if (ilvDev) {
-            GA_HIP(hipStreamSynchronize(stream));
+            syncStream();
             dfree(ilvDev, ilvBytes);
           }
           ilvBytes = need + need / 4;
@@ -156,7 +159,7 @@
                                   sizeof(float) * (size_t)(sg.b1 - sg.b0) * kBlock, kind, stream));
       }
     }
-    GA_HIP(hipStreamSynchronize(stream));
+    syncStream();
     doneBlocks += done;
   }
   if (blockCount > 0) freeRetired();
@@ -183,18 +186,19 @@
     Context& c;
     const bool blocking;
     ~Drain() {
-      if (blocking && c.stream) (void)hipStreamSynchronize(c.stream);
+      if (blocking) c.syncStreamQuiet();
       if (blocking && c.copyStream) (void)hipStreamSynchronize(c.copyStream);
     }
   } drain{*this, !pipelined.callerAsync};
   int64_t written = 0;
   if (cachedFrames > 0) {
     if (channels > cachedCh) fail(GA_ERR_OUT_OF_RANGE, "channelIndex");
+    joinTail();
     int toCopy = (int)std::min<int64_t>(cachedFrames, frameCount);
     for (int ch = 0; ch < channels; ch++)
       GA_HIP(hipMemcpyAsync(out[ch] + startIndex, cacheDev + (size_t)ch * kBlock + (kBlock - cachedFrames), sizeof(float) * toCopy,
                             kind, stream));
-    if (!asyncMode) GA_HIP(hipStreamSynchronize(stream));
+    if (!asyncMode) syncStream();
     written = toCopy;
     cachedFrames -= toCopy;
   }
@@ -221,7 +225,10 @@
     }
     struct Target {
       Context& c;
-      ~Target() { std::memset(c.busTarget, 0, sizeof(c.busTarget)); }
+      ~Target() {
+        std::memset(c.busTarget, 0, sizeof(c.busTarget));
+        c.tailWanted = false;
+      }
     } target{*this};
     const bool defer = direct && !deviceOut && pipelined.callerAsync && hostDefer && ownStream;
     if (defer) {
@@ -229,7 +236,7 @@
       if (deferStageBytes < rowBytes * 32) {
         flushHandOver();
         if (deferStage) {
-          GA_HIP(hipStreamSynchronize(stream));
+          syncStream();
           dfree(deferStage, deferStageBytes);
         }
         deferStageBytes = rowBytes * 32;
@@ -239,7 +246,9 @@
     } else if (direct) {
       for (int ch = 0; ch < channels; ch++) busTarget[ch] = tgt[ch];
     }
+    tailWanted = defer && coarseTailStream && !comm;
     runChunk(nblk, nullptr);
+    tailWanted = false;
     if (defer)
       for (int ch = 0; ch < channels; ch++)
         pendingHandOver.push_back(HandOver{busTarget[ch], tgt[ch], out[ch] + startIndex + written, chunkBlocksDone * kBlock});
@@ -264,11 +273,11 @@
                               hipMemcpyDeviceToDevice, stream));
       cachedFrames = (int)excess;
     }
-    if (!asyncMode) GA_HIP(hipStreamSynchronize(stream));
+    if (!asyncMode) syncStream();
     written += toCopy;
   }
   if (!pipelined.callerAsync) {
-    GA_HIP(hipStreamSynchronize(stream));
+    syncStream();
     harvestProfile(true);
     freeRetired();
   }
@@ -373,6 +382,11 @@
     else if (k == "conv_reference_order") c.convRefOrder = (int)std::min(2.0, std::max(0.0, value));
     else if (k == "conv_ref_min_deviation") c.convRefMinDeviation = std::max(0.0, value);
     else if (k == "coarse_premix") c.coarsePremix = value != 0;
+    else if (k == "coarse_tail_stream") c.coarseTailStream = value != 0;
+    else if (k == "coarse_premix_wgs_per_cu") {
+      if (!(value >= 1 && value <= 8) || value != (int)value) fail(GA_ERR_OUT_OF_RANGE, "coarse_premix_wgs_per_cu is 1 .. 8");
+      c.coarsePremixWgsPerCu = (int)value;
+    }
     else if (k == "coarse_long") c.coarseLong = value != 0;
     else if (k == "coarse_ext_history") c.coarseExtHist = value != 0;
     else if (k == "coarse_wide") c.coarseWide = value != 0;
@@ -420,7 +434,7 @@
 int ga_context_set_stream(ga_context* ctx, void* hip_stream) {
   return guard(ctx, [&](Context& c) {
     c.flushHandOver();
-    GA_HIP(hipStreamSynchronize(c.stream));
+    c.syncStream();
     c.waitHostCopies();
     if (c.ownStream && c.stream) (void)hipStreamDestroy(c.stream);
     c.stream = (hipStream_t)hip_stream;
@@ -450,7 +464,7 @@
       if (frames)
         GA_HIP(hipMemcpyAsync(b->dev + (size_t)i * b->stride, planar[i], sizeof(float) * frames, hipMemcpyHostToDevice, c.stream));
     }
-    GA_HIP(hipStreamSynchronize(c.stream));
+    c.syncStream();
     c.buffers.push_back(std::move(b));
     c.bufVersion++;
     *out_id = (int)c.buffers.size() - 1;
diff --git a/graphaudio_amd/csrc/ga_chunk.cpp b/graphaudio_amd/csrc/ga_chunk.cpp
--- a/graphaudio_amd/csrc/ga_chunk.cpp
+++ b/graphaudio_amd/csrc/ga_chunk.cpp
@@ -26,7 +26,7 @@
 void resetSlabs(Context& c, int64_t frames) {
   int64_t need = roundup(frames, 256);
   if (need > c.slabFrames) {
-    GA_HIP(hipStreamSynchronize(c.stream));
+    c.syncStream();
     size_t oldBytes = (size_t)c.slabFrames * sizeof(float);
     for (void* p : c.slabBlocks) c.dfree(p, oldBytes * slabsPerBlock(oldBytes));
     c.slabBlocks.clear();
@@ -202,7 +202,7 @@
       StereoPannerS& nd = rec<StereoPannerS>(*np);
       if (!nd.params[0].events.empty() || !nd.params[0].modulation.empty()) continue;
       PanState tmp;
-      GA_HIP(hipStreamSynchronize(stream));
+      syncStream();
       GA_HIP(hipMemcpy(&tmp, nd.panDev, sizeof(PanState), hipMemcpyDeviceToHost));
       nd.panLast = tmp.last_pan;
       nd.panGL = tmp.gain_l;
@@ -214,7 +214,7 @@
       if (spatialSignalDriven(nd)) continue;
       if (nd.spPrev.valid && nd.spCarry[nd.spCarryCur]) {
         SpatialCarry tmp;
-        GA_HIP(hipStreamSynchronize(stream));
+        syncStream();
         GA_HIP(hipMemcpy(&tmp, nd.spCarry[nd.spCarryCur], sizeof(SpatialCarry), hipMemcpyDeviceToHost));
         for (int q = 0; q < 4; q++) {
           nd.spPrev.idx[q] = tmp.idx[q];
@@ -239,7 +239,7 @@
       for (auto& p : nd.params) automated = automated || !p.events.empty() || !p.modulation.empty();
       if (!automated) {
         BiquadDynState tmp;
-        GA_HIP(hipStreamSynchronize(stream));
+        syncStream();
         GA_HIP(hipMemcpy(&tmp, nd.bqDyn, 24, hipMemcpyDeviceToHost));
         nd.b0 = tmp.b0; nd.b1 = tmp.b1; nd.b2 = tmp.b2; nd.a1 = tmp.a1; nd.a2 = tmp.a2;
         nd.coefDirty = tmp.dirty != 0;
@@ -479,7 +479,7 @@
       GA_HIP(hipMemsetAsync(nh, 0, maxD * rings * sizeof(float), stream));
       if (nd.delayHist) {
         GA_HIP(hipMemcpyAsync(nh, nd.delayHist, maxD * nd.delayHistRings * sizeof(float), hipMemcpyDeviceToDevice, stream));
-        GA_HIP(hipStreamSynchronize(stream));
+        syncStream();
         dfree(nd.delayHist, maxD * nd.delayHistRings * sizeof(float));
       }
       nd.delayHist = nh;
@@ -488,7 +488,7 @@
     const int64_t cap = roundup(frames, 4096);
     if (nd.delayCap < cap || nd.delayLineRings < rings) {
       if (nd.delayLine) {
-        GA_HIP(hipStreamSynchronize(stream));
+        syncStream();
         dfree(nd.delayLine, (maxD + (size_t)nd.delayCap) * nd.delayLineRings * sizeof(float));
       }
       nd.delayCap = std::max(nd.delayCap, cap);
@@ -502,7 +502,7 @@
   if (r.stage != 2) resetSlabs(*this, frames);
   if (zerosLen < frames) {
     if (zeros) {
-      GA_HIP(hipStreamSynchronize(stream));
+      syncStream();
       dfree(zeros, (size_t)zerosLen * 4);
     }
     zerosLen = roundup(frames, 4096);
@@ -510,7 +510,7 @@
     GA_HIP(hipMemsetAsync(zeros, 0, (size_t)zerosLen * 4, stream));
   }
   if (busCapFrames < frames) {
-    GA_HIP(hipStreamSynchronize(stream));
+    syncStream();
     for (float* p : busSlabs) dfree(p, (size_t)busCapFrames * 4);
     busSlabs.clear();
     busCapFrames = roundup(frames, 4096);
@@ -546,17 +546,28 @@
   if (asyncMode && chunkDone[slot]) GA_HIP(hipEventSynchronize(chunkDone[slot]));
   if (thostBytes < tbytes) {
     if (thost) {
-      GA_HIP(hipStreamSynchronize(stream));
+      syncStream();
       (void)hipHostFree(thost);
     }
     thostBytes = (tbytes + tbytes / 4 + 4096 + 15) & ~(size_t)15;
     GA_HIP(hipHostMalloc(&thost, thostBytes, hipHostMallocDefault));
   }
-  ensure(tables, std::max(tablesHostBytes, tablesHostBBytes));
+  const bool tailChunk = tailWanted && tailCandidate && ex.plan.launches.size() == 2 && ex.plan.launches[0].kind == GA_STAGE_COARSE_SECTION &&
+                         ex.plan.launches[1].kind == LK_CINV;
+  tailCandidate = false;
+  if (tailChunk) ensureOverlapStream();
+  else joinTail();
+  DevArena& tdev = (tailWanted && slot) ? tablesB : tables;
+  ensure(tdev, std::max(tablesHostBytes, tablesHostBBytes));
   std::memcpy(thost, ex.plan.host.data(), tbytes);
-  if (tableUploadKernel) launch_table_upload(stream, tables.p, thost, tbytes);
-  else GA_HIP(hipMemcpyAsync(tables.p, thost, tbytes, hipMemcpyHostToDevice, stream));
-  uint8_t* base = (uint8_t*)tables.p;
+  if (tableUploadKernel) launch_table_upload(stream, tdev.p, thost, tbytes);
+  else GA_HIP(hipMemcpyAsync(tdev.p, thost, tbytes, hipMemcpyHostToDevice, stream));
+  uint8_t* base = (uint8_t*)tdev.p;
+  struct TailActive {
+    Context& c;
+    ~TailActive() { c.tailActive = false; }
+  } tailGuard{*this};
+  tailActive = tailChunk;
 
   std::vector<std::pair<hipEvent_t, hipEvent_t>> evs;
   std::vector<int> evKind;
@@ -570,14 +581,15 @@
   }
   for (auto& l : ex.plan.launches) {
     hipEvent_t e0 = nullptr, e1 = nullptr;
+    const hipStream_t ls = l.kind == LK_CINV ? tailStreamNow() : stream;
     if (profile) {
       GA_HIP(hipEventCreate(&e0));
       GA_HIP(hipEventCreate(&e1));
-      GA_HIP(hipEventRecord(e0, stream));
+      GA_HIP(hipEventRecord(e0, ls));
     }
     l.fn(base);
     if (profile) {
-      GA_HIP(hipEventRecord(e1, stream));
+      GA_HIP(hipEventRecord(e1, ls));
       evs.push_back({e0, e1});
       evKind.push_back(l.kind);
       evBytes.push_back(l.bytes);
@@ -596,25 +608,30 @@
     evBytes.push_back(x.bytes);
   }
   extraProf.clear();
-  if (profile) GA_HIP(hipEventRecord(evEnd, stream));
+  if (profile) GA_HIP(hipEventRecord(evEnd, tailStreamNow()));
   GA_HIP(hipGetLastError());
   r.tmLaunch = nowMs();
   if (profileNow) pendingProf.push_back(ProfBatch{evBegin, evEnd, std::move(evs), std::move(evKind), std::move(evBytes)});
   if (asyncMode) {
     if (!chunkDone[slot]) GA_HIP(hipEventCreateWithFlags(&chunkDone[slot], hipEventDisableTiming));
-    GA_HIP(hipEventRecord(chunkDone[slot], stream));
+    GA_HIP(hipEventRecord(chunkDone[slot], tailStreamNow()));
+    if (tailChunk) {
+      GA_HIP(hipEventRecord(tailEv, stream2));
+      tailPending = true;
+    }
     harvestProfile(false);
   } else {
-    GA_HIP(hipStreamSynchronize(stream));
+    syncStream();
     harvestProfile(true);
   }
+  tailActive = false;
   chunkSeq++;
   if (gaTiming)
     fprintf(stderr, "[ga]   host detail: topo %.2f, sources %.2f, sim %.2f | resources %.2f, params %.2f, exec %.2f ms\n", r.tmTopo - r.tm0,
             r.tmSrc - r.tmTopo, r.tmSim - r.tmSrc, r.tmRes - r.tmSim, r.tmPre - r.tmRes, r.tmPlan - r.tmPre);
   if (gaTiming)
-    fprintf(stderr, "[ga] chunk %lld blocks: sim %.2f ms, plan %.2f ms, enqueue %.2f ms, wait %.2f ms\n", (long long)n, r.tmSim - r.tm0,
-            r.tmPlan - r.tmSim, r.tmLaunch - r.tmPlan, nowMs() - r.tmLaunch);
+    fprintf(stderr, "[ga] chunk %lld blocks: sim %.2f ms, plan %.2f ms, enqueue %.2f ms, wait %.2f ms%s\n", (long long)n, r.tmSim - r.tm0,
+            r.tmPlan - r.tmSim, r.tmLaunch - r.tmPlan, nowMs() - r.tmLaunch, tailChunk ? ", coarse stage on the second stream" : "");
 
 }
 
@@ -813,7 +830,7 @@
   chunkExecute(r1);
   if (r1.waited) {
     const double tw0 = nowMs();
-    GA_HIP(hipStreamSynchronize(stream));
+    syncStream();
     if (gaTiming) fprintf(stderr, "[ga]   two-stage chunk: stage 1 wait %.3f ms\n", nowMs() - tw0);
   }
   for (int id : r1.probeDelays) {
@@ -957,7 +974,7 @@
   const size_t devBytes = readBytes + descCount * sizeof(GsrBlock);
   if (rateModDevBytes < devBytes) {
     if (rateModDev) {
-      GA_HIP(hipStreamSynchronize(stream));
+      syncStream();
       dfree(rateModDev, rateModDevBytes);
     }
     rateModDevBytes = devBytes + devBytes / 2 + 4096;
diff --git a/graphaudio_amd/csrc/ga_coarse.hip b/graphaudio_amd/csrc/ga_coarse.hip
--- a/graphaudio_amd/csrc/ga_coarse.hip
+++ b/graphaudio_amd/csrc/ga_coarse.hip
@@ -1257,14 +1257,11 @@
 #define GA_PREMIX_NT 0
 #endif
 constexpr int kPremixAhead = GA_PREMIX_AHEAD, kPremixWaves = GA_PREMIX_WAVES;
-#ifndef GA_PREMIX_WORDS
-#define GA_PREMIX_WORDS 1
-#endif
 #ifndef GA_PREMIX_COPY_WGS
 #define GA_PREMIX_COPY_WGS 8
 #endif
 constexpr int kPremixCopyWgs = GA_PREMIX_COPY_WGS;
-constexpr int kPremixWords = GA_PREMIX_WORDS, kPremixTile = 256 * kPremixWords;
+constexpr int kPremixStep = 64;
 struct Kahan4 {
   v4f s, c;
   __device__ __forceinline__ void add(v4f x) {
@@ -1278,9 +1275,8 @@
   }
 };
 template <bool ALIGNED, bool CARRY>
-__device__ __forceinline__ void premix_stream(const PremixJob& J, const PremixTerm* __restrict terms, int t0, int t1, int lane,
-                                              const uint32_t (&off)[kPremixWords], const bool (&keep)[kPremixWords],
-                                              const uint32_t (&coff)[kPremixWords], Kahan4 (&acc)[kPremixWords]) {
+__device__ __forceinline__ void premix_stream(const PremixJob& J, const PremixTerm* __restrict terms, int t0, int t1, int lane, uint32_t off, bool keep,
+                                              uint32_t coff, Kahan4& acc) {
   typedef const GA_GLOBAL char* gcp;
   typedef GA_GLOBAL char* gp;
   auto fetch = [&](gcp in, uint32_t o) -> v4f {
@@ -1309,46 +1305,38 @@
     };
     int j = 0;
     for (; j + kPremixAhead <= nb; j += kPremixAhead) {
-      v4f x[kPremixAhead][kPremixWords];
-#pragma unroll
-      for (int u = 0; u < kPremixAhead; u++) {
-        gcp in = in_of(j + u);
-#pragma unroll
-        for (int w = 0; w < kPremixWords; w++) x[u][w] = fetch(in, off[w]);
-      }
+      v4f x[kPremixAhead];
+#pragma unroll
+      for (int u = 0; u < kPremixAhead; u++) x[u] = fetch(in_of(j + u), off);
 #pragma unroll
       for (int u = 0; u < kPremixAhead; u++) {
         if (CARRY) {
           gp car = carry_of(j + u);
-#pragma unroll
-          for (int w = 0; w < kPremixWords; w++)
-            if (car && keep[w]) put(car, coff[w], x[u][w]);
+          if (car && keep) put(car, coff, x[u]);
         }
-#pragma unroll
-        for (int w = 0; w < kPremixWords; w++) acc[w].add(x[u][w]);
+        acc.add(x[u]);
       }
     }
     for (; j < nb; j++) {
       gcp in = in_of(j);
       gp car = CARRY ? carry_of(j) : nullptr;
-#pragma unroll
-      for (int w = 0; w < kPremixWords; w++) {
-        const v4f x = fetch(in, off[w]);
-        if (CARRY && car && keep[w]) put(car, coff[w], x);
-        acc[w].add(x);
-      }
-    }
-  }
-}
-__global__ __launch_bounds__(64 * kPremixWaves) void coarse_premix_kernel(const PremixJob* __restrict jobs, const PremixTerm* __restrict terms) {
-  __shared__ v4f part[kPremixWaves - 1][2][kPremixWords][64];
-  const PremixJob J = jobs[blockIdx.y];
-  if (J.flags & 4) {
-    if (blockIdx.x >= (unsigned)kPremixCopyWgs) return;
+      const v4f x = fetch(in, off);
+      if (CARRY && car && keep) put(car, coff, x);
+      acc.add(x);
+    }
+  }
+}
+__global__ __launch_bounds__(64 * kPremixWaves) void coarse_premix_kernel(const PremixJob* __restrict jobs, const PremixTerm* __restrict terms,
+                                                                          int n_handover, int wgs_per_job) {
+  __shared__ v4f part[2][kPremixWaves - 1][2][kPremixStep];
+  const unsigned copy_wgs = (unsigned)n_handover * kPremixCopyWgs;
+  if (blockIdx.x < copy_wgs) {
+    const PremixJob J = jobs[blockIdx.x / kPremixCopyWgs];
+    const unsigned wg = blockIdx.x % kPremixCopyWgs;
     const GA_GLOBAL v4f* src = (const GA_GLOBAL v4f*)terms[J.term0].in;
     GA_GLOBAL v4f* dst = (GA_GLOBAL v4f*)J.out;
     const int64_t nw = J.n / 4, step = (int64_t)kPremixCopyWgs * blockDim.x * 2;
-    for (int64_t i = (int64_t)blockIdx.x * blockDim.x * 2 + threadIdx.x; i < nw; i += step) {
+    for (int64_t i = (int64_t)wg * blockDim.x * 2 + threadIdx.x; i < nw; i += step) {
       const int64_t i2 = i + blockDim.x;
       const v4f a = src[i], b = i2 < nw ? src[i2] : a;
       dst[i] = a;
@@ -1356,58 +1344,66 @@
     }
     return;
   }
-  const int64_t tile0 = (int64_t)blockIdx.x * kPremixTile;
-  if (tile0 >= J.n) return;
+  const unsigned sb = blockIdx.x - copy_wgs;
+  const PremixJob J = jobs[n_handover + sb / (unsigned)wgs_per_job];
+  const int64_t nw = J.n / 4, lines = (nw + 7) / 8, wg = sb % (unsigned)wgs_per_job;
+  const int64_t w0 = lines * wg / wgs_per_job * 8, w1 = min(nw, lines * (wg + 1) / wgs_per_job * 8);
+  if (w0 >= w1) return;
   const int lane = threadIdx.x & 63, wv = __builtin_amdgcn_readfirstlane(threadIdx.x >> 6);
-  int64_t f[kPremixWords];
-  bool live[kPremixWords], keep[kPremixWords];
-  uint32_t off[kPremixWords], coff[kPremixWords];
-  Kahan4 acc[kPremixWords];
-#pragma unroll
-  for (int w = 0; w < kPremixWords; w++) {
-    f[w] = tile0 + (int64_t)(w * 64 + lane) * 4;
-    live[w] = f[w] < J.n;
-    keep[w] = live[w] && f[w] >= J.carry_from;
-    off[w] = live[w] ? (uint32_t)(f[w] * 4) : 0u;
-    coff[w] = (uint32_t)((f[w] - J.carry_from) * 4);
-    acc[w] = Kahan4{v4f{0.f, 0.f, 0.f, 0.f}, v4f{0.f, 0.f, 0.f, 0.f}};
-  }
   const int per = ((J.nterms + kPremixWaves - 1) / kPremixWaves + kPremixAhead - 1) / kPremixAhead * kPremixAhead;
   const int t0 = min(J.nterms, wv * per), t1 = min(J.nterms, t0 + per);
-  const bool carry_here = (J.flags & 2) && tile0 + kPremixTile > J.carry_from;
-  if (J.flags & 1) {
-    if (carry_here) premix_stream<true, true>(J, terms, t0, t1, lane, off, keep, coff, acc);
-    else premix_stream<true, false>(J, terms, t0, t1, lane, off, keep, coff, acc);
-  } else {
-    if (carry_here) premix_stream<false, true>(J, terms, t0, t1, lane, off, keep, coff, acc);
-    else premix_stream<false, false>(J, terms, t0, t1, lane, off, keep, coff, acc);
-  }
-  if (wv > 0) {
-#pragma unroll
-    for (int w = 0; w < kPremixWords; w++) {
-      part[wv - 1][0][w][lane] = acc[w].s;
-      part[wv - 1][1][w][lane] = acc[w].c;
-    }
-  }
-  __syncthreads();
-  if (wv == 0) {
-#pragma unroll
-    for (int w = 0; w < kPremixWords; w++) {
+  int buf = 0;
+  for (int64_t ws = w0; ws < w1; ws += kPremixStep, buf ^= 1) {
+    const int64_t f = (ws + lane) * 4;
+    const bool live = ws + lane < w1, keep = live && f >= J.carry_from;
+    const uint32_t off = (uint32_t)((live ? f : ws * 4) * 4);
+    const uint32_t coff = (uint32_t)((f - J.carry_from) * 4);
+    Kahan4 acc{v4f{0.f, 0.f, 0.f, 0.f}, v4f{0.f, 0.f, 0.f, 0.f}};
+    const bool carry_here = (J.flags & 2) && (ws + kPremixStep) * 4 > J.carry_from;
+    if (J.flags & 1) {
+      if (carry_here) premix_stream<true, true>(J, terms, t0, t1, lane, off, keep, coff, acc);
+      else premix_stream<true, false>(J, terms, t0, t1, lane, off, keep, coff, acc);
+    } else {
+      if (carry_here) premix_stream<false, true>(J, terms, t0, t1, lane, off, keep, coff, acc);
+      else premix_stream<false, false>(J, terms, t0, t1, lane, off, keep, coff, acc);
+    }
+    if (wv > 0) {
+      part[buf][wv - 1][0][lane] = acc.s;
+      part[buf][wv - 1][1][lane] = acc.c;
+    }
+    __syncthreads();
+    if (wv == 0) {
 #pragma unroll
       for (int q = 0; q < kPremixWaves - 1; q++) {
-        acc[w].add(part[q][0][w][lane]);
-        acc[w].add(-part[q][1][w][lane]);
-      }
-      if (live[w]) stg4(J.out + f[w], acc[w].s);
-    }
-  }
-}
-const char* launch_coarse_premix(hipStream_t s, const PremixJob* jobs_dev, int njobs, const PremixTerm* terms_dev, int64_t max_n) {
+        acc.add(part[buf][q][0][lane]);
+        acc.add(-part[buf][q][1][lane]);
+      }
+      if (live) stg4(J.out + f, acc.s);
+    }
+  }
+}
+static int premix_compute_units() {
+  static int cached[64];
+  int dev = 0;
+  if (hipGetDevice(&dev) != hipSuccess || dev < 0 || dev >= 64) launch_fail("coarse pre-mix: no current device");
+  if (!cached[dev]) {
+    hipDeviceProp_t prop;
+    if (hipGetDeviceProperties(&prop, dev) != hipSuccess) launch_fail("coarse pre-mix: no device properties");
+    cached[dev] = std::max(1, prop.multiProcessorCount);
+  }
+  return cached[dev];
+}
+const char* launch_coarse_premix(hipStream_t s, const PremixJob* jobs_dev, int njobs, int n_handover, const PremixTerm* terms_dev, int64_t max_n,
+                                 int wgs_per_cu) {
   if (njobs <= 0 || max_n <= 0) return "";
-  const int64_t gx = (max_n + kPremixTile - 1) / kPremixTile;
-  if (gx > 0x7fffffff || max_n >= ((int64_t)1 << 29)) launch_fail("coarse pre-mix: chunk too long");
-  for (int j0 = 0; j0 < njobs; j0 += 32768)
-    hipLaunchKernelGGL(coarse_premix_kernel, dim3((unsigned)gx, std::min(32768, njobs - j0)), dim3(64 * kPremixWaves), 0, s, jobs_dev + j0, terms_dev);
+  if (max_n >= ((int64_t)1 << 29)) launch_fail("coarse pre-mix: chunk too long");
+  if (n_handover < 0 || n_handover > njobs || wgs_per_cu < 1) launch_fail("coarse pre-mix: bad launch parameters");
+  const int nsum = njobs - n_handover;
+  const int64_t steps = (max_n / 4 + kPremixStep - 1) / kPremixStep;
+  const int per_job = nsum ? (int)std::max<int64_t>(1, std::min<int64_t>(steps, (int64_t)wgs_per_cu * premix_compute_units() / nsum)) : 1;
+  const int64_t grid = (int64_t)n_handover * kPremixCopyWgs + (int64_t)nsum * per_job;
+  if (grid > 0x7fffffff) launch_fail("coarse pre-mix: too many jobs");
+  hipLaunchKernelGGL(coarse_premix_kernel, dim3((unsigned)grid), dim3(64 * kPremixWaves), 0, s, jobs_dev, terms_dev, n_handover, per_job);
   return "coarse_premix_kernel";
 }
 
diff --git a/graphaudio_amd/csrc/ga_comm.cpp b/graphaudio_amd/csrc/ga_comm.cpp
--- a/graphaudio_amd/csrc/ga_comm.cpp
+++ b/graphaudio_amd/csrc/ga_comm.cpp
@@ -119,6 +119,7 @@
 }
 
 void Context::commWait() {
+  joinTail();
   if (!comm) {
     GA_HIP(hipStreamSynchronize(stream));
     return;
@@ -180,11 +181,12 @@
       if (!out[ch]) fail(GA_ERR_INVALID_ARGUMENT, "Channel buffer is null.");
   }
   GA_HIP(hipSetDevice(device));
+  joinTail();
   const size_t need_ = (size_t)channels * (size_t)frames * sizeof(float);
   if (reduceBytes < need_) {
     flushHandOver();
     if (reduceBuf) {
-      GA_HIP(hipStreamSynchronize(stream));
+      syncStream();
       dfree(reduceBuf, reduceBytes);
     }
     reduceBytes = need_ + need_ / 8;
diff --git a/graphaudio_amd/csrc/ga_engine.cpp b/graphaudio_amd/csrc/ga_engine.cpp
--- a/graphaudio_amd/csrc/ga_engine.cpp
+++ b/graphaudio_amd/csrc/ga_engine.cpp
@@ -160,7 +160,7 @@
 void Context::ensure(DevArena& a, size_t bytes) {
   if (a.bytes >= bytes) return;
   if (a.p) {
-    GA_HIP(hipStreamSynchronize(stream));
+    syncStream();
     dfree(a.p, a.bytes);
     a.p = nullptr;
     a.bytes = 0;
@@ -193,6 +193,7 @@
 
 Context::~Context() {
   if (stream) (void)hipStreamSynchronize(stream);
+  if (stream2) (void)hipStreamSynchronize(stream2);
   try {
     commDestroy();
   } catch (...) {
@@ -263,6 +264,8 @@
     for (auto& e : dGroupEv)
       if (e) (void)hipEventDestroy(e);
     if (dJoinEv) (void)hipEventDestroy(dJoinEv);
+    if (tailEv) (void)hipEventDestroy(tailEv);
+    if (premixEv) (void)hipEventDestroy(premixEv);
   }
   for (auto& x : extraProf) { (void)hipEventDestroy(x.e0); (void)hipEventDestroy(x.e1); }
   if (coarseX.p) (void)hipFree(coarseX.p);
@@ -281,6 +284,7 @@
   for (float* p : bqSplitBlocks) (void)hipFree(p);
   if (ilvDev) (void)hipFree(ilvDev);
   if (tables.p) (void)hipFree(tables.p);
+  if (tablesB.p) (void)hipFree(tablesB.p);
   if (tablesHost) (void)hipHostFree(tablesHost);
   if (tablesHostB) (void)hipHostFree(tablesHostB);
   for (auto& e : chunkDone)
@@ -373,7 +377,7 @@
         continue;
       }
       if (!synced && stream) {
-        (void)hipStreamSynchronize(stream);
+        syncStreamQuiet();
         synced = true;
       }
       PlayBuf& b = *buffers[id];
@@ -387,7 +391,7 @@
   }
   for (auto it = irCache.begin(); it != irCache.end();) {
     if (it->second.use_count() == 1) {
-      if (stream) (void)hipStreamSynchronize(stream);
+      syncStreamQuiet();
       it = irCache.erase(it);
     } else {
       ++it;
@@ -425,7 +429,23 @@
     pendingProf.pop_front();
   }
 }
+void Context::joinTail() {
+  if (!tailPending) return;
+  GA_HIP(hipStreamWaitEvent(stream, tailEv, 0));
+  tailPending = false;
+}
+void Context::syncStream() {
+  joinTail();
+  GA_HIP(hipStreamSynchronize(stream));
+}
+void Context::syncStreamQuiet() {
+  if (!stream) return;
+  if (tailPending) (void)hipStreamWaitEvent(stream, tailEv, 0);
+  tailPending = false;
+  (void)hipStreamSynchronize(stream);
+}
 void Context::flushHandOver() {
+  joinTail();
   for (const HandOver& h : pendingHandOver)
     GA_HIP(hipMemcpyAsync(h.dst_host, h.src, sizeof(float) * (size_t)h.n, hipMemcpyDeviceToHost, stream));
   pendingHandOver.clear();
@@ -462,7 +482,7 @@
     if (outPending[k]) GA_HIP(hipEventSynchronize(outCopied[k]));
     outPending[k] = false;
     if (outStage[k]) {
-      GA_HIP(hipStreamSynchronize(stream));
+      syncStream();
       dfree(outStage[k], outStageBytes[k]);
       outStage[k] = nullptr;
       outStageBytes[k] = 0;
@@ -553,7 +573,7 @@
   for (int p = 0; p < (int)n.params.size(); p++) inputDisconnectAll(InRef{id, -1 - p});
   if (n.type == GA_NODE_DELAY) {
     DelayS& d = rec<DelayS>(n);
-    if (stream) (void)hipStreamSynchronize(stream);
+    syncStreamQuiet();
     if (d.delayHist) dfree(d.delayHist, (size_t)d.maxDelaySamples * d.delayHistRings * sizeof(float));
     if (d.delayLine) dfree(d.delayLine, ((size_t)d.maxDelaySamples + (size_t)d.delayCap) * d.delayLineRings * sizeof(float));
     d.delayHist = d.delayLine = nullptr;
@@ -561,7 +581,7 @@
     d.delayCap = 0;
   }
   if (n.staleBuf) {
-    if (stream) (void)hipStreamSynchronize(stream);
+    syncStreamQuiet();
     dfree(n.staleBuf, (size_t)n.staleRows * kBlock * sizeof(float));
     dfree(n.staleNext, (size_t)n.staleRows * kBlock * sizeof(float));
     n.staleBuf = n.staleNext = nullptr;
@@ -570,21 +590,21 @@
   if (n.type == GA_NODE_SPATIAL_PANNER) {
     SpatialPannerS& sp = rec<SpatialPannerS>(n);
     if (sp.spHist[0]) {
-      if (stream) (void)hipStreamSynchronize(stream);
+      syncStreamQuiet();
       for (float*& h : sp.spHist) {
         dfree(h, kSpatialMaxTaps * sizeof(float));
         h = nullptr;
       }
     }
     if (sp.spCarry[0]) {
-      if (stream) (void)hipStreamSynchronize(stream);
+      syncStreamQuiet();
       for (SpatialCarry*& h : sp.spCarry) {
         dfree(h, sizeof(SpatialCarry));
         h = nullptr;
       }
     }
     if (sp.spDirect) {
-      if (stream) (void)hipStreamSynchronize(stream);
+      syncStreamQuiet();
       dfree(sp.spDirect, sizeof(SpatialDirectState));
       sp.spDirect = nullptr;
     }
@@ -614,7 +634,7 @@
     if (r.group) r.group->rows[r.idx] = {-1, 0};
   n.convRows.clear();
   if (n.bHistR || n.bOverlap) {
-    if (stream) (void)hipStreamSynchronize(stream);
+    syncStreamQuiet();
     if (n.ir) {
       size_t hb = (size_t)n.bInCh * kBins * std::max(n.ir->P - 1, 1) * sizeof(float);
       dfree(n.bHistR, hb);
@@ -626,13 +646,13 @@
     dfree(n.bOverlap, (size_t)n.bSlots * 2 * kBlock * sizeof(float));
   }
   if (n.dHist[0]) {
-    if (stream) (void)hipStreamSynchronize(stream);
+    syncStreamQuiet();
     dfree(n.dHistBase[0], n.dHistBytes);
     dfree(n.dHistBase[1], n.dHistBytes);
     n.dHistBase[0] = n.dHistBase[1] = nullptr;
   }
   if (n.dTail[0]) {
-    if (stream) (void)hipStreamSynchronize(stream);
+    syncStreamQuiet();
     for (int b = 0; b < 2; b++) dfree(n.dTail[b], (size_t)n.dTailLen * n.dTailCh * sizeof(float));
   }
   n.dTail[0] = n.dTail[1] = nullptr;
@@ -680,7 +700,7 @@
   memcpy(tab, jobs.data(), jobs.size() * sizeof(HistJobB));
   launch_hist_copy_b(stream, tab, (int)jobs.size(), maxh);
   GA_HIP(hipGetLastError());
-  GA_HIP(hipStreamSynchronize(stream));
+  syncStream();
   GA_HIP(hipHostFree(tab));
 }
 
@@ -986,13 +1006,13 @@
     std::vector<ConvRowIO> r2(nch);
     for (int c = 0; c < nch; c++) r2[c] = ConvRowIO{dIn + (size_t)c * padded + (size_t)t0 * kBlock, nullptr};
     if (t0 > 0) {
-      GA_HIP(hipStreamSynchronize(stream));
+      syncStream();
       GA_HIP(hipMemcpy(rowsDev, r2.data(), sizeof(ConvRowIO) * nch, hipMemcpyHostToDevice));
     }
     launch_rfft_fwd(stream, rowsDev, nch, nb, t0, pl, Twiddles{w128, w256});
   }
   launch_extract_ir(stream, sp->hr, sp->hi, xr, xi, P, rp, P, nch);
-  GA_HIP(hipStreamSynchronize(stream));
+  syncStream();
   GA_HIP(hipGetLastError());
   sp->taps = dIn;
   sp->tapsStride = padded;
@@ -1041,6 +1061,8 @@
   GA_HIP(hipStreamCreateWithFlags(&stream2, hipStreamNonBlocking));
   for (auto& e : dGroupEv) GA_HIP(hipEventCreateWithFlags(&e, hipEventDisableTiming));
   GA_HIP(hipEventCreateWithFlags(&dJoinEv, hipEventDisableTiming));
+  GA_HIP(hipEventCreateWithFlags(&tailEv, hipEventDisableTiming));
+  GA_HIP(hipEventCreateWithFlags(&premixEv, hipEventDisableTiming));
 }
 const float2* Context::coarseTwab() {
   if (coarseTw) return coarseTw;
@@ -1083,7 +1105,7 @@
   GA_HIP(hipMemcpy(rd, rows.data(), sizeof(CoarseXRow) * rows.size(), hipMemcpyHostToDevice));
   launch_coarse_fwd(stream, rd, ir.nch, P, P, ir.coarse, twiddles16pw(), coarseTwab());
   GA_HIP(hipGetLastError());
-  GA_HIP(hipStreamSynchronize(stream));
+  syncStream();
   dfree(rd, sizeof(CoarseXRow) * rows.size());
 }
 
diff --git a/graphaudio_amd/csrc/ga_engine.hpp b/graphaudio_amd/csrc/ga_engine.hpp
--- a/graphaudio_amd/csrc/ga_engine.hpp
+++ b/graphaudio_amd/csrc/ga_engine.hpp
@@ -835,6 +835,17 @@
   void handOverToHost(const float* const* src, float* const* out, int channels, int64_t offset, int64_t frames);
   void waitHostCopies();
   hipStream_t stream2 = nullptr;
+  bool coarseTailStream = true;
+  bool tailWanted = false;
+  bool tailCandidate = false;
+  bool tailActive = false;
+  bool tailPending = false;
+  hipEvent_t tailEv = nullptr, premixEv = nullptr;
+  DevArena tablesB;
+  void joinTail();
+  void syncStream();
+  void syncStreamQuiet();
+  hipStream_t tailStreamNow() const { return tailActive ? stream2 : stream; }
   hipEvent_t dGroupEv[8] = {nullptr, nullptr, nullptr, nullptr, nullptr, nullptr, nullptr, nullptr};
   hipEvent_t dJoinEv = nullptr;
   bool coarseOverlap = false;
@@ -855,6 +866,7 @@
   bool coarseCarry = true;
   bool coarseLong = true;
   bool coarsePremix = true;
+  int coarsePremixWgsPerCu = 2;
   void ensureOverlapStream();
   void noteKernel(int kind, const char* name) {
     if (kind < 0 || kind >= 16 || !name || !*name) return;
diff --git a/graphaudio_amd/csrc/ga_kernels.hpp b/graphaudio_amd/csrc/ga_kernels.hpp
--- a/graphaudio_amd/csrc/ga_kernels.hpp
+++ b/graphaudio_amd/csrc/ga_kernels.hpp
@@ -169,7 +169,8 @@
   int flags;
   int pad_;
 };
-const char* launch_coarse_premix(hipStream_t s, const PremixJob* jobs_dev, int njobs, const PremixTerm* terms_dev, int64_t max_n);
+const char* launch_coarse_premix(hipStream_t s, const PremixJob* jobs_dev, int njobs, int n_handover, const PremixTerm* terms_dev, int64_t max_n,
+                                 int wgs_per_cu);
 const char* launch_coarse_fwd(hipStream_t s, const CoarseXRow* rows_dev, int nrows, int max_frames, int run, float2* X, const float2* tw16,
                        const float2* twab, const CoarseHandOver* handover_dev = nullptr, int n_handover = 0);
 const char* launch_coarse_mac(hipStream_t s, const CoarseJob* jobs_dev, int njobs, const CoarseTerm* terms_dev, const float2* X, float2* Y,
diff --git a/graphaudio_amd/csrc/ga_plan_conv.cpp b/graphaudio_amd/csrc/ga_plan_conv.cpp
--- a/graphaudio_amd/csrc/ga_plan_conv.cpp
+++ b/graphaudio_amd/csrc/ga_plan_conv.cpp
@@ -25,7 +25,7 @@
                               hipMemcpyDeviceToDevice, c.stream));
     }
     GA_HIP(hipMemcpyAsync(o0, g.overlap[g.ovCur], (size_t)g.rp * kBlock * 4, hipMemcpyDeviceToDevice, c.stream));
-    GA_HIP(hipStreamSynchronize(c.stream));
+    c.syncStream();
     size_t oldH = (size_t)kBins * std::max(hist, 1) * g.rp * sizeof(float);
     c.dfree(g.histR, oldH);
     c.dfree(g.histI, oldH);
@@ -170,6 +170,7 @@
   std::vector<PremixTerm> pmTerms;
   size_t pmUsed = 0;
   int64_t pmMaxN = 0;
+  int pmHandOver = 0;
   double pmBytes = 0;
   std::vector<CoarseXRow> xrows;
   std::vector<CoarseHistJob> hjobs;
@@ -394,8 +395,9 @@
     int xFrame[32], xIndex[32];
     for (int ch = 0; ch < g.nxr; ch++) {
       const size_t bytes = (size_t)(hl + frames) * sizeof(float);
-      if (pmUsed + bytes > c.coarseM.bytes) fail(GA_ERR_INVALID_OPERATION, "internal: the pre-mix arena is too small for the plan");
-      float* mixed = (float*)((char*)c.coarseM.p + pmUsed);
+      const size_t half = (c.coarseM.bytes / 2) & ~(size_t)255;
+      if (pmUsed + bytes > half) fail(GA_ERR_INVALID_OPERATION, "internal: the pre-mix arena is too small for the plan");
+      float* mixed = (float*)((char*)c.coarseM.p + ((c.chunkSeq & 1) ? half : 0) + pmUsed);
       pmUsed += (bytes + 255) & ~(size_t)255;
       auto job = [&](float* out, const std::vector<PremixTerm>& tv, int64_t len, int64_t carryFrom) {
         PremixJob j{out, (int)pmTerms.size(), 0, len, carryFrom, 1, 0};
@@ -435,7 +437,12 @@
     addPieces(ld, kv.first, g.nxr, xFrame, xIndex);
     c.stats.coarse_premixed_signals += (int64_t)g.members * g.nxr;
   }
-  if (!pmJobs.empty() && !c.pendingHandOver.empty()) {
+  c.tailCandidate = c.tailWanted && !pmJobs.empty() && hjobs.empty() && !c.coarseOverlap && ex.plan.launches.empty();
+  if (c.tailCandidate && !c.pendingHandOver.empty() && !xrows.empty()) {
+    for (const Context::HandOver& h : c.pendingHandOver) fwdHandOver.push_back(CoarseHandOver{h.src, h.dst_dev, h.n});
+    c.pendingHandOver.clear();
+    c.stats.deferred_handovers++;
+  } else if (!pmJobs.empty() && !c.pendingHandOver.empty()) {
     std::vector<PremixJob> head;
     for (const Context::HandOver& h : c.pendingHandOver) {
       head.push_back(PremixJob{h.dst_dev, (int)pmTerms.size(), 1, h.n, h.n, 1 | 4, 0});
@@ -444,6 +451,7 @@
       pmBytes += 2.0 * (double)h.n * 4.0;
     }
     pmJobs.insert(pmJobs.begin(), head.begin(), head.end());
+    pmHandOver = (int)head.size();
     c.pendingHandOver.clear();
     c.stats.deferred_handovers++;
   } else if (!c.pendingHandOver.empty() && !xrows.empty()) {
@@ -583,7 +591,7 @@
       if (nch == 0) continue;
       if (!ld.dTail[0] || ld.dTailLen != len || ld.dTailCh != nch) {
         if (kv.second.carried) fail(GA_ERR_INVALID_OPERATION, "internal: a carried tail changed its shape");
-        GA_HIP(hipStreamSynchronize(c.stream));
+        c.syncStream();
         for (int b = 0; b < 2; b++) {
           if (ld.dTail[b]) c.dfree(ld.dTail[b], (size_t)ld.dTailLen * ld.dTailCh * sizeof(float));
           ld.dTail[b] = (float*)c.dalloc((size_t)len * nch * sizeof(float));
@@ -636,7 +644,7 @@
   const size_t xo = ex.plan.putv(xrows), ho = ex.plan.putv(hjobs), to = ex.plan.putv(terms), oo = ex.plan.putv(outs), yo = ex.plan.putv(ylist);
   const size_t pjo = ex.plan.putv(pmJobs), pto = ex.plan.putv(pmTerms), fho = ex.plan.putv(fwdHandOver);
   const int nfh = (int)fwdHandOver.size();
-  const int npm = (int)pmJobs.size();
+  const int npm = (int)pmJobs.size(), npmHandOver = this->pmHandOver, pmWgsPerCu = c.coarsePremixWgsPerCu;
   const int64_t pmMaxN = this->pmMaxN;
   const double pmBytes = this->pmBytes, pmFlops = this->pmFlops, invFlops = this->invFlops;
   struct MacLaunch { size_t off; int nj, cw, mt, mp, pb, grp; bool ap; double bytes, flops; };
@@ -694,18 +702,23 @@
       cp->stats.stage_bytes[kind] += bytes;
       cp->stats.stage_flops[kind] += flops;
     };
-    hipStream_t s2 = G > 1 ? cp->stream2 : st;
     if (npm > 0)
-      timed(st, LK_CPREMIX, pmBytes, pmFlops, [&] { return launch_coarse_premix(st, (const PremixJob*)(base + pjo), npm, (const PremixTerm*)(base + pto), pmMaxN); });
+      timed(cp->stream, LK_CPREMIX, pmBytes, pmFlops, [&] { return launch_coarse_premix(st, (const PremixJob*)(base + pjo), npm, npmHandOver, (const PremixTerm*)(base + pto), pmMaxN, pmWgsPerCu); });
+    hipStream_t ts = cp->tailStreamNow();
+    if (cp->tailActive) {
+      GA_HIP(hipEventRecord(cp->premixEv, cp->stream));
+      GA_HIP(hipStreamWaitEvent(ts, cp->premixEv, 0));
+    }
+    hipStream_t s2 = G > 1 ? cp->stream2 : ts;
     for (int g = 0; g < G; g++) {
       const FwdLaunch& f = fwds[g];
       if (f.nx > 0)
-        timed(st, LK_CFWD, f.bytes, f.flops, [&] {
-          return launch_coarse_fwd(st, (const CoarseXRow*)(base + xo) + f.x0, f.nx, f.maxFrames, f.run, X, twFwd, twab,
+        timed(ts, LK_CFWD, f.bytes, f.flops, [&] {
+          return launch_coarse_fwd(ts, (const CoarseXRow*)(base + xo) + f.x0, f.nx, f.maxFrames, f.run, X, twFwd, twab,
                                    (const CoarseHandOver*)(base + fho), g == 0 ? nfh : 0);
         });
       if (G > 1) {
-        GA_HIP(hipEventRecord(cp->dGroupEv[g], st));
+        GA_HIP(hipEventRecord(cp->dGroupEv[g], ts));
         GA_HIP(hipStreamWaitEvent(s2, cp->dGroupEv[g], 0));
       }
       for (const MacLaunch& m : macs)
@@ -717,11 +730,11 @@
     }
     if (G > 1) {
       GA_HIP(hipEventRecord(cp->dJoinEv, s2));
-      GA_HIP(hipStreamWaitEvent(st, cp->dJoinEv, 0));
+      GA_HIP(hipStreamWaitEvent(ts, cp->dJoinEv, 0));
     }
   });
   ex.plan.add(LK_CINV, [=](uint8_t* base) {
-    cp->noteKernel(LK_CINV, launch_coarse_inv(st, (const CoarseOut*)(base + oo), no, invBlocks, (const int*)(base + yo), Y, yFrames, tw16, twab));
+    cp->noteKernel(LK_CINV, launch_coarse_inv(cp->tailStreamNow(), (const CoarseOut*)(base + oo), no, invBlocks, (const int*)(base + yo), Y, yFrames, tw16, twab));
   }, invBytes, invFlops);
   const int64_t mh = maxHist;
   if (nh > 0) ex.plan.add(LK_CHIST, [=](uint8_t* base) { launch_coarse_hist(st, (const CoarseHistJob*)(base + ho), nh, mh); }, histBytes);
@@ -1016,7 +1029,7 @@
         }
         size_t pm = 0;
         for (auto& kv : pmDepth) pm = std::max(pm, kv.second);
-        if (pm) ensure(coarseM, pm);
+        if (pm) ensure(coarseM, 2 * pm + 512);
       }
     }
     bRowX = bRowY = 0;
diff --git a/graphaudio_amd/csrc/ga_plan_nodes.cpp b/graphaudio_amd/csrc/ga_plan_nodes.cpp
--- a/graphaudio_amd/csrc/ga_plan_nodes.cpp
+++ b/graphaudio_amd/csrc/ga_plan_nodes.cpp
@@ -734,7 +734,7 @@
       init.dirty = nd.coefDirty ? 1 : 0;
       nd.coefDirty = false;
       GA_HIP(hipMemcpyAsync(nd.bqDyn, &init, 24, hipMemcpyHostToDevice, stream));
-      GA_HIP(hipStreamSynchronize(stream));
+      syncStream();
       nd.coefOnDevice = true;
       deviceStateNodes.push_back(ns.id);
     }
@@ -1036,7 +1036,7 @@
     const int rows = nd.type == GA_NODE_CHANNEL_SPLITTER ? std::max<int>(1, (int)nd.outputs.size()) : 32;
     if (!nd.staleBuf || nd.staleRows < rows) {
       if (nd.staleBuf) {
-        GA_HIP(hipStreamSynchronize(stream));
+        syncStream();
         dfree(nd.staleBuf, (size_t)nd.staleRows * kBlock * sizeof(float));
         dfree(nd.staleNext, (size_t)nd.staleRows * kBlock * sizeof(float));
       }
```

New measurement: 1.300 billion (median of 6 runs). 1.06x the previous value.
